# ctSkennerton/crass

Hardware: AMD Instinct MI355X
Metric: reads/sec through DR search+recruit, 150bp synthetic, 1/2/4/8 MI355X (higher is better)
Workload: dtype u8; 1 GPU; 100000000 synthetic 150 bp reads, 50 seeded DRs, 1 % CRISPR reads (BASELINE.json configs[2]); pass1 + merge + pass2; total_reads=100000000, reads_per_gpu=100000000, read_len=150, n_dr=50, parallelism=read-shards x1, launcher=single context, pass1_found=563794, pass2_found=436000, patterns=13320, ac_states=0, filter_survivors=1705594, fast_filter=1, lds_automaton=2, merge_fallbacks=0

## Files before the change

### crass_amd/build.py

```python
import os
import shutil
import subprocess
import sys

HERE = os.path.dirname(os.path.abspath(__file__))
CSRC = os.path.join(HERE, "csrc")
LIB = os.path.join(HERE, "libcrass_hip.so")
SOURCES = ["kernels.hip", "pass2.hip", "sinks.hip", "dmerge.hip", "consensus.hip", "pack.hip", "fastx_scan.hip", "fastx_names.hip", "inflate.hip", "gunzip.hip", "engine.cpp", "engine_pass1.cpp", "engine_merge.cpp", "engine_pass2.cpp", "engine_ingest.cpp", "merge.cpp", "ingest.cpp", "fastx_scan.cpp", "bgzf.cpp", "gunzip.cpp", "consensus.cpp", "group.cpp", "graph.cpp", "sdma.cpp", "pgzip.cpp"]
HEADERS = ["engine_internal.h", "engine_ctx.h", "dev_common.h", "comp_table.h", "devmem.h", "pack_text.h", "lane_find.h", "pack_launch.h", "fastx_scan.h", "fastx_launch.h", "fastx_shards.h", "fastx_names_launch.h", "inflate_core.h", "inflate_launch.h", "gunzip_core.h", "gunzip_launch.h", "consensus_internal.h", "merge.h", os.path.join("..", "..", "include", "crass_hip.h")]


def _hipcc():
    for cand in (os.environ.get("HIPCC"), shutil.which("hipcc"), "/opt/rocm/bin/hipcc"):
        if cand and os.path.exists(cand):
            return cand
    raise RuntimeError("hipcc not found: the MI355X engine cannot be built")


OBJ = os.path.join(CSRC, "_obj")
FLAGS = ["--offload-arch=gfx950", "-O3", "-std=c++17", "-ffp-contract=off", "-fPIC", "-Wall", "-Wno-unused-function"]
LIBS = ["-lz", "-lpthread", "-ldl"]


def _stale(target, deps):
    if not os.path.exists(target):
        return True
    t = os.path.getmtime(target)
    return any(os.path.getmtime(d) > t for d in deps)


def needs_build():
    return _stale(LIB, [os.path.join(CSRC, d) for d in SOURCES + HEADERS])


def build(force=False, verbose=False):
    if not force and not needs_build():
        return LIB
    os.makedirs(OBJ, exist_ok=True)
    hipcc = _hipcc()
    hdrs = [os.path.join(CSRC, h) for h in HEADERS]
    jobs = []
    objs = []
    for s in SOURCES:
        src, obj = os.path.join(CSRC, s), os.path.join(OBJ, s + ".o")
        objs.append(obj)
        if force or _stale(obj, [src] + hdrs):
            cmd = [hipcc] + FLAGS + ["-x", "hip", "-c", src, "-o", obj]
            if verbose:
                print(" ".join(cmd), file=sys.stderr)
            jobs.append((s, subprocess.Popen(cmd, stdout=subprocess.PIPE, stderr=subprocess.STDOUT, text=True)))
    failed = []
    for s, p in jobs:
        out, _ = p.communicate()
        if out.strip():
            print(out, file=sys.stderr, end="")
        if p.returncode:
            failed.append(s)
    if failed:
        raise RuntimeError("hipcc failed for: " + ", ".join(failed))
    tmp = LIB + ".tmp"
    cmd = [hipcc, "--offload-arch=gfx950", "-shared", "-fPIC", "-o", tmp] + objs + LIBS
    if verbose:
        print(" ".join(cmd), file=sys.stderr)
    subprocess.check_call(cmd)
    from . import vgpr_guard
    try:
        vgpr_guard.check(tmp)
    except Exception:
        os.replace(tmp, LIB + ".rejected")
        raise
    os.replace(tmp, LIB)
    return LIB


ADAPTER_DIR = os.path.join(CSRC, "adapter")
CLI = os.path.join(HERE, "crass-hip")
ADAPTER_LIB = os.path.join(HERE, "libcrass_adapter.so")


def build_adapter(force=False, verbose=False):
    build(force=force, verbose=verbose)
    srcs = [os.path.join(ADAPTER_DIR, "crass_adapter.cpp")]
    deps = srcs + [os.path.join(ADAPTER_DIR, "crass_adapter.h"), os.path.join(ADAPTER_DIR, "crass_hip_cli.cpp"), LIB]
    if not force and os.path.exists(CLI) and os.path.exists(ADAPTER_LIB) and \
            all(os.path.getmtime(d) <= min(os.path.getmtime(CLI), os.path.getmtime(ADAPTER_LIB)) for d in deps):
        return CLI
    cxx = shutil.which("g++") or "g++"
    common = [cxx, "-O2", "-std=c++17", "-Wall", "-fPIC", "-pthread"]
    rpath = ["-L" + HERE, "-lcrass_hip", "-Wl,-rpath," + HERE, "-Wl,-rpath,$ORIGIN"]
    for cmd in (common + ["-shared", "-o", ADAPTER_LIB] + srcs + rpath,
                common + ["-o", CLI, os.path.join(ADAPTER_DIR, "crass_hip_cli.cpp")] + srcs + rpath):
        if verbose:
# ... 9 lines not shown
```

### crass_amd/csrc/dev_common.h

```cpp
#pragma once
#include "engine_internal.h"

namespace crass {

#define WAVE 64

static __device__ __forceinline__ void wave_sync()
{
    __builtin_amdgcn_fence(__ATOMIC_RELEASE, "wavefront");
    __builtin_amdgcn_wave_barrier();
    __builtin_amdgcn_fence(__ATOMIC_ACQUIRE, "wavefront");
}

static __device__ __forceinline__ uint32_t uni(uint32_t x) { return (uint32_t)__builtin_amdgcn_readfirstlane((int)x); }
static __device__ __forceinline__ int uni(int x) { return __builtin_amdgcn_readfirstlane(x); }
static __device__ __forceinline__ uint64_t uni64(uint64_t x) { return ((uint64_t)uni((uint32_t)(x >> 32)) << 32) | (uint64_t)uni((uint32_t)x); }

static __device__ __forceinline__ uint64_t rd_word_off(const DevReads &R, uint64_t r)
{
    return R.stride_words ? r * (uint64_t)R.stride_words : R.word_off[r];
}
static __device__ __forceinline__ uint32_t rd_len(const DevReads &R, uint64_t r)
{
    return R.uniform_len ? R.uniform_len : R.lengths[r];
}
static __device__ __forceinline__ bool rd_is_exc(const DevReads &R, uint64_t r)
{
    return (R.exc_mask[r >> 5] >> (r & 31)) & 1u;
}
static __device__ __forceinline__ uint64_t rd_hint_off(const DevReads &R, uint64_t r)
{
    return R.uniform_len ? r * (uint64_t)((R.uniform_len + 63u) >> 6) : R.pos_hint_off[r];
}
static __device__ __forceinline__ uint64_t rd_header_id(const DevReads &R, uint64_t r)
{
    return R.header_id ? R.header_id[r] : r;
}

typedef unsigned short u16x2 __attribute__((ext_vector_type(2)));
static __device__ __forceinline__ uint32_t pk_min_u16(uint32_t a, uint32_t b)
{
    u16x2 r = __builtin_elementwise_min(__builtin_bit_cast(u16x2, a), __builtin_bit_cast(u16x2, b));
    return __builtin_bit_cast(uint32_t, r);
}

}
```

### crass_amd/csrc/dmerge.hip

```cpp
#include "engine_internal.h"
#include <algorithm>

namespace crass {

#define WAVE 64
static constexpr uint32_t kUnres = 0xFFFFFFFFu;
static constexpr uint32_t kNoLane = 0xFFFFFFFEu;
static constexpr int kClusterK = 11;

static __device__ __forceinline__ uint64_t shr128_lo(uint64_t h0, uint64_t h1, uint32_t bits)
{
    if (bits == 0) return h0;
    if (bits < 64) return (h0 >> bits) | (h1 << (64 - bits));
    return h1 >> (bits - 64);
}
static __device__ __forceinline__ uint64_t shr128_hi(uint64_t h1, uint32_t bits)
{
    return bits < 64 ? (h1 >> bits) : 0ull;
}
static __device__ __forceinline__ void mask128(uint32_t len, uint64_t &m0, uint64_t &m1)
{
    if (len >= 32) { m0 = ~0ull; m1 = len >= 64 ? ~0ull : ((1ull << (2 * (len - 32))) - 1ull); }
    else { m0 = (1ull << (2 * len)) - 1ull; m1 = 0ull; }
}
// ... 835 lines not shown

static __device__ __forceinline__ uint32_t dm_rd_len(const DevReads &R, uint64_t r) { return R.uniform_len ? R.uniform_len : R.lengths[r]; }
static __device__ __forceinline__ uint64_t dm_rd_off(const DevReads &R, uint64_t r) { return R.stride_words ? r * (uint64_t)R.stride_words : R.word_off[r]; }

#define DV_MAXW 20
#define DV_G 3
#define DV_GL 21

template <typename WordFn>
static __device__ __forceinline__ void dv_candidates(const DevMerge &M, WordFn word, const uint8_t *raw, uint32_t L, uint32_t a, uint32_t cnt_s,
                                                     uint32_t base_s, int lane, uint32_t &best_end, uint32_t &best_len, uint32_t &best_pid)
{
    for (uint32_t c0 = 0; c0 < cnt_s; c0 += 64) {
        const uint32_t c = c0 + lane;
        uint32_t cand = 0xFFFFFFFFu, cpid = 0;
        if (c < cnt_s) {
            const uint64_t *ent = M.ents + (uint64_t)(base_s + c) * 2;
            const uint64_t *ent2 = M.ents + ((uint64_t)M.ent_cap + base_s + c) * 2;
            const uint64_t e0 = ent[0], e1 = ent[1], f0 = ent2[0], f1 = ent2[1];
            const uint32_t rr = (uint32_t)e0 & 7u, len = ((uint32_t)e0 >> 3) & 0x7Fu;
            if (a >= rr && a - rr + len <= L) {
                const uint32_t start = a - rr;
                const uint32_t w0 = start >> 4, sh = (start & 15u) * 2u;
                uint32_t x[5];
#pragma unroll
                for (int q = 0; q < 5; q++) x[q] = word(w0 + q);
                uint32_t y[4];
#pragma unroll
                for (int q = 0; q < 4; q++) y[q] = sh ? ((x[q] >> sh) | (x[q + 1] << (32 - sh))) : x[q];
                const uint64_t v0 = (uint64_t)y[0] | ((uint64_t)y[1] << 32), v1 = (uint64_t)y[2] | ((uint64_t)y[3] << 32);
                uint64_t m0, m1;
                mask128(len, m0, m1);
                bool eq = (v0 & m0) == e1 && (v1 & m1) == f0;
                const uint64_t e_mask = f1;
                if (eq && raw) {
                    uint64_t rm = 0;
                    bool other = false;
                    for (uint32_t i = 0; i < len; i++) {
                        const uint8_t ch = raw[start + i];
                        if (!((ch == 'A') | (ch == 'C') | (ch == 'G') | (ch == 'T'))) { rm |= 1ull << i; other |= ch != 'N'; }
                    }
                    eq = !other && rm == e_mask;
                } else if (eq) eq = e_mask == 0ull;
                if (eq) { cand = ((start + len) << 8) | (255u - len); cpid = (uint32_t)(e0 >> 32); }
            }
        }
        uint32_t mn = cand;
#pragma unroll
        for (int off = 32; off > 0; off >>= 1) mn = min(mn, (uint32_t)__shfl_xor((int)mn, off));
        if (mn != 0xFFFFFFFFu) {
            const uint32_t e_end = mn >> 8, e_len = 255u - (mn & 0xFFu);
            if (e_end < best_end || (e_end == best_end && e_len > best_len)) {
                const uint64_t who = __ballot(cand == mn);
                best_end = e_end; best_len = e_len;
                best_pid = (uint32_t)__shfl((int)cpid, __ffsll((unsigned long long)who) - 1);
            }
        }
    }
}

static __device__ __forceinline__ void dv_probe(const DevMerge &M, uint32_t V, uint32_t kmask, uint32_t &cnt, uint32_t &base)
{
    const unsigned long long want = (unsigned long long)V | (1ull << 32);
    uint32_t s = kset_hash(V, M.kset_log);
    for (;;) {
        const unsigned long long kk = M.kset_key[s];
        const uint32_t c_s = M.kset_cnt[s], b_s = M.kset_base[s];
        if (kk == 0ull) break;
        if (kk == want) { cnt = c_s; base = b_s; break; }
        s = (s + 1) & kmask;
    }
}

static __device__ __forceinline__ const uint8_t *dv_raw(const DevReads &R, uint64_t r)
{
    if (!(R.n_exc && ((R.exc_mask[r >> 5] >> (r & 31)) & 1u))) return nullptr;
    uint64_t lo = 0, hi = R.n_exc - 1;
    while (lo < hi) { const uint64_t mid = (lo + hi) >> 1; if (R.exc_read[mid] < r) lo = mid + 1; else hi = mid; }
    return R.exc_bytes + R.exc_off[lo];
}

template <bool SHORT, int U>
__global__ __launch_bounds__(256) void k_dm_verify(DevReads R, DevMerge M, const uint64_t *idx, const uint32_t *d_n, uint64_t n_max,
                                                    uint32_t *info_by_slot, uint32_t *pid_by_slot)
{
    __shared__ uint32_t rw_all[4][DV_G][DV_MAXW + 2];
    const int lane = threadIdx.x & 63, wv = threadIdx.x >> 6;
    const uint64_t wave = __builtin_amdgcn_readfirstlane((uint32_t)((blockIdx.x * (uint64_t)blockDim.x + threadIdx.x) >> 6));
    const uint64_t n_waves = ((uint64_t)gridDim.x * blockDim.x) >> 6;
    uint64_t n = *d_n;
    if (n > n_max) n = n_max;
    const uint32_t kmask = (1u << M.kset_log) - 1u;
    if (SHORT) {
        const int gi = lane / DV_GL, pl = lane % DV_GL;
        const uint32_t L = R.uniform_len, nw = (L + 15) >> 4, h_max = (L - 16) >> 3;
        const bool grp = gi < DV_G;
        const uint64_t stride = n_waves * DV_G;
        const int g0 = (grp ? gi : 0) * DV_GL;
        const uint64_t gmask = grp ? (((1ull << DV_GL) - 1ull) << g0) : 0ull;
        uint32_t *rw = rw_all[wv][grp ? gi : 0];
        const ulonglong2 *ents1 = reinterpret_cast<const ulonglong2 *>(M.ents), *ents2 = ents1 + M.ent_cap;
        uint64_t k = wave * DV_G + (uint64_t)gi;
        bool have = grp && k < n;
        uint64_t r = have ? idx[k] : 0;
        uint32_t wreg = (have && (uint32_t)pl < nw) ? R.packed[dm_rd_off(R, r) + pl] : 0u;
        uint64_t k_n = k + stride;
        bool have_n = grp && k_n < n;
        uint64_t r_n = have_n ? idx[k_n] : 0;
        for (uint64_t k0 = wave * DV_G; k0 < n; k0 += stride) {
            if (have && (uint32_t)pl <= nw + 4u) rw[pl] = wreg;
            __builtin_amdgcn_fence(__ATOMIC_RELEASE, "wavefront");
            __builtin_amdgcn_wave_barrier();
            __builtin_amdgcn_fence(__ATOMIC_ACQUIRE, "wavefront");
            const uint32_t wreg_n = (have_n && (uint32_t)pl < nw) ? R.packed[dm_rd_off(R, r_n) + pl] : 0u;
            const uint64_t k_nn = k_n + stride;
            const bool have_nn = grp && k_nn < n;
            const uint64_t r_nn = have_nn ? idx[k_nn] : 0;
            uint32_t cnt = 0, base = 0;
            if (have && (uint32_t)pl <= h_max) {
                const uint32_t wi = (uint32_t)pl >> 1;
                const uint32_t lo = rw[wi], hi = rw[wi + 1];
                dv_probe(M, (pl & 1) ? ((lo >> 16) | (hi << 16)) : lo, kmask, cnt, base);
            }
            const uint8_t *raw = nullptr;
            if (R.n_exc && have) raw = dv_raw(R, r);
            const uint64_t hits_all = __ballot(cnt > 0);
            uint32_t my = grp ? (uint32_t)(hits_all >> (gi * DV_GL)) & ((1u << DV_GL) - 1u) : 0u;
            uint32_t be = 0xFFFFFFFFu, bl = 0, bp = 0;
            while (__ballot(my != 0u)) {
                bool act = my != 0u;
                const int wsrc = act ? __ffs((int)my) - 1 : 0;
                if (act) my &= my - 1u;
                const uint32_t a = 8u * (uint32_t)wsrc;
                if (act && be <= a + 15u) { act = false; my = 0u; }
                const uint32_t cnt_s = (uint32_t)__shfl((int)cnt, g0 + wsrc), base_s = (uint32_t)__shfl((int)base, g0 + wsrc);
                for (uint32_t c0 = 0; __ballot(act && c0 < cnt_s); c0 += U * DV_GL) {
                    uint32_t cand = 0xFFFFFFFFu, cpid = 0;
                    uint32_t cq[U];
                    bool vq[U];
                    ulonglong2 e1[U], e2[U];
#pragma unroll
                    for (int q = 0; q < U; q++) {
                        cq[q] = c0 + (uint32_t)(q * DV_GL + pl);
                        vq[q] = act && cq[q] < cnt_s;
                        const uint32_t ei = vq[q] ? base_s + cq[q] : 0u;
                        e1[q] = ents1[ei]; e2[q] = ents2[ei];
                    }
#pragma unroll
                    for (int q = 0; q < U; q++) {
                        const uint64_t e0 = e1[q].x;
                        const uint32_t rr = (uint32_t)e0 & 7u, len = ((uint32_t)e0 >> 3) & 0x7Fu;
                        if (vq[q] && a >= rr && a - rr + len <= L) {
                            const uint32_t start = a - rr;
                            const uint32_t w0 = start >> 4, sh = (start & 15u) * 2u;
                            uint32_t x[5];
#pragma unroll
                            for (int i = 0; i < 5; i++) x[i] = rw[w0 + i];
                            uint32_t y[4];
#pragma unroll
                            for (int i = 0; i < 4; i++) y[i] = __builtin_amdgcn_alignbit(x[i + 1], x[i], sh);
                            const uint64_t v0 = (uint64_t)y[0] | ((uint64_t)y[1] << 32), v1 = (uint64_t)y[2] | ((uint64_t)y[3] << 32);
                            uint64_t m0, m1;
                            mask128(len, m0, m1);
                            bool eq = (v0 & m0) == e1[q].y && (v1 & m1) == e2[q].x;
                            const uint64_t e_mask = e2[q].y;
                            if (eq && raw) {
                                uint64_t rm = 0;
                                bool other = false;
                                for (uint32_t i = 0; i < len; i++) {
                                    const uint8_t ch = raw[start + i];
                                    if (!((ch == 'A') | (ch == 'C') | (ch == 'G') | (ch == 'T'))) { rm |= 1ull << i; other |= ch != 'N'; }
                                }
                                eq = !other && rm == e_mask;
                            } else if (eq) eq = e_mask == 0ull;
// ... 7 lines not shown
                        uint32_t mn = cand;
#pragma unroll
                        for (int off = 16; off > 0; off >>= 1) {
                            const uint32_t o = (uint32_t)__shfl_down((int)mn, off);
                            if (pl + off < DV_GL) mn = min(mn, o);
                        }
                        mn = (uint32_t)__shfl((int)mn, g0);
                        const uint64_t who = __ballot(cand == mn) & gmask;
                        const uint32_t pid = (uint32_t)__shfl((int)cpid, who ? __ffsll((unsigned long long)who) - 1 : 0);
                        const uint32_t e_end = mn >> 8, e_len = 255u - (mn & 0xFFu);
                        if (e_end < be || (e_end == be && e_len > bl)) { be = e_end; bl = e_len; bp = pid; }
                    }
                }
            }
            if (have && pl == 0) {
                info_by_slot[k] = bl ? ((be << 8) | bl) : 0u;
                pid_by_slot[k] = bp;
            }
            __builtin_amdgcn_wave_barrier();
            k = k_n; have = have_n; r = r_n; wreg = wreg_n;
            k_n = k_nn; have_n = have_nn; r_n = r_nn;
        }
        return;
    }
    uint32_t *rw = rw_all[wv][0];
    for (uint64_t k = wave; k < n; k += n_waves) {
        const uint64_t r = idx[k];
        const uint32_t L = dm_rd_len(R, r);
        const uint32_t *g = R.packed + dm_rd_off(R, r);
        const uint32_t nw = (L + 15) >> 4;
        const bool staged = nw <= DV_MAXW;
        const uint8_t *raw = dv_raw(R, r);
        if (staged) {
            if ((uint32_t)lane < nw) rw[lane] = g[lane];
            if ((uint32_t)lane == nw) rw[lane] = 0u;
            __builtin_amdgcn_fence(__ATOMIC_RELEASE, "wavefront");
            __builtin_amdgcn_wave_barrier();
            __builtin_amdgcn_fence(__ATOMIC_ACQUIRE, "wavefront");
        }
        auto word = [&](uint32_t i) -> uint32_t {
            if (staged) return rw[min(i, nw)];
            return i < nw ? g[i] : 0u;
        };
        uint32_t best_end = 0xFFFFFFFFu, best_len = 0, best_pid = 0;
        const uint32_t KL = M.akey_bases, vmask = akey_mask(M);
        if (L >= KL) {
            const uint32_t ash = M.akey_shift;
            const uint32_t h_max = (L - KL) >> ash;
            for (uint32_t hb = 0; hb <= h_max; hb += 64) {
                if (best_end <= (hb << ash) + KL - 1u) break;
                const uint32_t h = hb + lane;
                uint32_t cnt = 0, base = 0;
                if (h <= h_max) {
                    const uint32_t pos = h << ash, wi = pos >> 4;
                    const uint32_t lo = word(wi), hi = word(wi + 1);
                    dv_probe(M, __builtin_amdgcn_alignbit(hi, lo, (pos & 15u) * 2u) & vmask, kmask, cnt, base);
                }
                uint64_t hits = __ballot(cnt > 0);
                while (hits) {
                    const int src = __ffsll((unsigned long long)hits) - 1;
                    hits &= hits - 1;
                    const uint32_t a = (hb + (uint32_t)src) << ash;
                    if (best_end <= a + KL - 1u) { hits = 0; break; }
                    const uint32_t cnt_s = (uint32_t)__shfl((int)cnt, src), base_s = (uint32_t)__shfl((int)base, src);
                    dv_candidates(M, word, raw, L, a, cnt_s, base_s, lane, best_end, best_len, best_pid);
                }
            }
        }
        if (lane == 0) {
            info_by_slot[k] = best_len ? ((best_end << 8) | best_len) : 0u;
            pid_by_slot[k] = best_pid;
        }
        __builtin_amdgcn_wave_barrier();
    }
}

hipError_t warm_dmerge_module()
{
    hipFuncAttributes a;
    return hipFuncGetAttributes(&a, reinterpret_cast<const void *>(&k_xg_unpack));
}

hipError_t launch_dm_verify(const DevReads &R, const DevMerge &M, const uint64_t *idx, const uint32_t *d_n, uint64_t n_max,
                            uint32_t *info_by_slot, uint32_t *pid_by_slot, hipStream_t st)
{
    if (n_max == 0) return hipSuccess;
    static const bool dv_one = getenv("CRASS_DV_ONE") != nullptr;
    const bool shortr = M.akey_shift == 3 && M.akey_bases == 16 && R.uniform_len >= 16 && ((R.uniform_len - 16) >> 3) < DV_GL && ((R.uniform_len + 15) >> 4) <= DV_MAXW && !dv_one;
    uint64_t nb = shortr ? (n_max + 4 * DV_G - 1) / (4 * DV_G) : (n_max + 3) / 4;
    if (nb > 8192) nb = 8192;
    static const bool dv_pair = getenv("CRASS_DV_SINGLE") == nullptr;
    if (shortr && dv_pair) CRASS_LAUNCH((k_dm_verify<true, 2>), dim3((unsigned)nb), dim3(256), 0, st, R, M, idx, d_n, n_max, info_by_slot, pid_by_slot);
    else if (shortr) CRASS_LAUNCH((k_dm_verify<true, 1>), dim3((unsigned)nb), dim3(256), 0, st, R, M, idx, d_n, n_max, info_by_slot, pid_by_slot);
    else CRASS_LAUNCH((k_dm_verify<false, 1>), dim3((unsigned)nb), dim3(256), 0, st, R, M, idx, d_n, n_max, info_by_slot, pid_by_slot);
    return hipGetLastError();
}

}
```

### crass_amd/csrc/engine.cpp

```cpp
#include "engine_ctx.h"

#include <cstdio>
#include <new>
#include <string>

void crass_hip_ctx::widen_p1() const
{
    P1Dense &D = dense;
    if (D.wide_ready) return;
    (void)wait_bulk();
    const uint64_t n = D.n;
    const uint32_t ss_cap = D.pack_ss_cap, stride = dr_stride;
    const uint8_t *hb = D.h_blob.p;
    const uint16_t *b_replen = (const uint16_t *)(hb + D.lay.replen), *b_ss = (const uint16_t *)(hb + D.lay.ss);
    const uint8_t *b_nss = hb + D.lay.nss, *b_ss8 = hb + D.lay.ss;
    D.w_replen.resize(n); D.w_nss.resize(n); D.w_ss_off.resize(n); D.w_ss.resize(n * (size_t)ss_cap);
    D.w_dr_len.resize(n); D.w_dr.resize(n * (size_t)stride);
    if (D.dr_fallback) (void)hipStreamSynchronize(copy_stream);
    else (void)wait_dx();
    const size_t per_task = 16384;
    host_parallel_for((size_t)((n + per_task - 1) / per_task), 16, [&](size_t t) {
        const uint64_t k0 = t * per_task, k1 = std::min<uint64_t>(n, k0 + per_task);
        for (uint64_t k = k0; k < k1; k++) { D.w_replen[k] = b_replen[k]; D.w_nss[k] = b_nss[k]; D.w_ss_off[k] = k * (uint64_t)ss_cap; }
        if (D.lay.ss_elem == 1) for (uint64_t i = k0 * ss_cap; i < k1 * (uint64_t)ss_cap; i++) D.w_ss[i] = b_ss8[i];
// ... 118 lines not shown
    c->poll_on = getenv("CRASS_NO_POLL") == nullptr;
    if (hipEventCreateWithFlags(&c->ev_gathered, hipEventDisableTiming) != hipSuccess) { delete c; return CRASS_ERR_HIP; }
    if (hipEventCreateWithFlags(&c->ev_premerge, hipEventDisableTiming) != hipSuccess) { delete c; return CRASS_ERR_HIP; }
    c->dma = sdma_create();
    if (c->dma && !getenv("CRASS_DX_PINNED")) {
        for (auto &d : c->dma_dx) d = sdma_create();
        c->dx_via_dma = c->dma_dx[0] && c->dma_dx[1] && c->dma_dx[2];
    }
    (void)warm_dmerge_module();
    *out = c;
    return CRASS_OK;
}

int crass_hip_stream_wait_event(crass_hip_ctx *c, void *event)
{
    if (!c || !event) return CRASS_ERR_INVALID_ARG;
    (void)hipSetDevice(c->device);
    HIPCHK(c, hipStreamWaitEvent(c->stream, (hipEvent_t)event, 0));
    return CRASS_OK;
}

int crass_hip_reload_env(crass_hip_ctx *c)
{
    if (!c) return CRASS_ERR_INVALID_ARG;
    c->env.read();
    g_dev_cap.store(c->env.pool_cap_bytes, std::memory_order_relaxed);
    c->dp.debug_stop = c->env.surv_debug;
    c->dp.find_serial = c->env.lane_find_serial ? 1u : 0u;
    if (c->env.stage_timing >= 0) c->timing_level = c->env.stage_timing;
    c->lb_on = !c->env.no_lookback;
    return CRASS_OK;
}

int crass_hip_set_stage_timing(crass_hip_ctx *c, int level)
{
    if (!c || level < 0 || level > 2) return CRASS_ERR_INVALID_ARG;
    c->timing_level = level;
    return CRASS_OK;
}

int crass_hip_set_host_view(crass_hip_ctx *c, int light)
{
    if (!c || light < 0 || light > 1) return CRASS_ERR_INVALID_ARG;
    quiesce_worker(c);
    c->host_view_light = light != 0;
    if (c->host_view_light) c->dm.M.x_on = 0;
    return CRASS_OK;
}

int crass_hip_set_timing_focus(crass_hip_ctx *c, unsigned kernels)
{
    if (!c || kernels > 7u) return CRASS_ERR_INVALID_ARG;
    c->timing_focus = kernels;
    return CRASS_OK;
}

void crass_hip_destroy(crass_hip_ctx *c)
{
    if (!c) return;
    (void)hipSetDevice(c->device);
    quiesce_worker(c);
    c->worker.stop();
    if (c->stream) (void)hipStreamSynchronize(c->stream);
    if (c->copy_stream) (void)hipStreamSynchronize(c->copy_stream);
    if (c->hint_stream) (void)hipStreamSynchronize(c->hint_stream);
    (void)sdma_wait(c->dma);
    (void)c->wait_dx();
    ingest_free_all(c);
    if (getenv("CRASS_POLL_REPORT")) fprintf(stderr, "[crass_hip] stage-flag polls that ran out of their budget: %u (of %u flags)\n", c->n_poll_timeouts.load(), c->flag_seq);
    c->lb_status.release(); c->lb_ticket.release(); c->h_lb_fail.release(); c->h_flags.release();
    if (c->xchg.ev_counts) (void)hipEventDestroy(c->xchg.ev_counts);
    c->dm.release(); c->h_qblob.release(); c->xchg.send.release(); c->xchg.xinfo.release(); c->xchg.h_xinfo.release();
    c->dd_map.release(); c->dd_dx_chars.release(); c->dd_dx_len.release(); c->dd_dx_hash.release();
    c->h_dmap.release(); c->h_dx_chars.release(); c->h_dx_len.release(); c->h_dx_hash.release();
    if (c->ev_gathered) (void)hipEventDestroy(c->ev_gathered);
    if (c->ev_sink_copies) (void)hipEventDestroy(c->ev_sink_copies);
    for (int q = 0; q < crass_hip_ctx::kHintParts; q++) if (c->ev_hint[q]) (void)hipEventDestroy(c->ev_hint[q]);
    if (c->ev_hint_go) (void)hipEventDestroy(c->ev_hint_go);
    if (c->hint_stream) (void)hipStreamDestroy(c->hint_stream);
    sdma_destroy(c->dma); c->dma = nullptr;
    for (auto &d : c->dma_sink) { sdma_destroy(d); d = nullptr; }
    for (auto &d : c->dma_dx) { sdma_destroy(d); d = nullptr; }
    if (c->ev_premerge) (void)hipEventDestroy(c->ev_premerge);
    if (c->copy_stream) (void)hipStreamDestroy(c->copy_stream);
    c->r_packed.release(); c->r_word_off.release(); c->r_lengths.release(); c->r_header_id.release();
    c->r_exc_mask.release(); c->r_exc_read.release(); c->r_exc_off.release(); c->r_exc_bytes.release();
    c->d_mask.release(); c->d_word_prefix.release(); c->d_block_sums.release(); c->d_idx.release(); c->d_count.release();
    c->d_found.release(); c->d_hit_info.release(); c->d_surv.release(); c->d_dr.release(); c->d_ss_pool.release();
    c->d_ss_used.release(); c->d_rec.release(); c->d_exc_hit.release(); c->d_extra.release();
    c->g_surv.release(); c->g_dr.release(); c->g_ss.release(); c->g_fidx.release(); c->h_count.release(); c->h_surv.release(); c->h_dr.release(); c->h_ss.release(); c->h_idx.release(); c->h_rec.release();
    c->a_go4w.release(); c->a_go16.release(); c->a_go32.release(); c->a_out.release(); c->a_go4.release(); c->dense.release(); c->d_fidx.release(); c->d_pos_hint.release(); c->d_pos_hint_off.release(); c->d_pos_hint_blk.release(); c->d_punt.release(); c->d_redo.release(); c->dd_keys.release(); c->dd_first.release(); c->dd_slot.release(); c->dd_rep.release(); c->dd_hash.release(); c->h_rep.release(); c->h_hash.release(); c->a_anchor.release(); c->d_slot_info.release(); c->d_slot_pid.release(); c->a_out_pid.release(); c->a_pat_token.release();
    for (auto &e : c->ev) if (e) (void)hipEventDestroy(e);
    if (c->stream) (void)hipStreamDestroy(c->stream);
    delete c;
}

int validate_reads(const crass_reads *r)
{
    if (!r) return CRASS_ERR_INVALID_ARG;
    if (r->n_reads && !r->packed) return CRASS_ERR_INVALID_ARG;
    if (!r->stride_words && r->n_reads && !r->word_off) return CRASS_ERR_INVALID_ARG;
    if (!r->uniform_len && r->n_reads && !r->lengths) return CRASS_ERR_INVALID_ARG;
    if (r->n_exceptions && (!r->exc_read || !r->exc_off || !r->exc_bytes)) return CRASS_ERR_INVALID_ARG;
    if (r->uniform_len > CRASS_HIP_MAX_READ_LEN) return CRASS_ERR_UNSUPPORTED;
    return CRASS_OK;
}

int alloc_scratch(crass_hip_ctx *c)
{
    const uint64_t n = c->R.n_reads;
    const uint64_t n_words = std::max<uint64_t>((n + 63) / 64, 1024);
    HIPCHK(c, c->d_mask.ensure(n_words + 1));
    HIPCHK(c, c->d_word_prefix.ensure(n_words + 1));
    HIPCHK(c, c->d_block_sums.ensure((n_words + 255) / 256 + 2));
    HIPCHK(c, c->d_idx.ensure(n + 1));
    HIPCHK(c, c->d_count.ensure(8));
    HIPCHK(c, c->d_found.ensure(n + 1));
    HIPCHK(c, c->d_hit_info.ensure(n + 1));
    HIPCHK(c, c->d_ss_used.ensure(4));
    HIPCHK(c, c->h_count.ensure(32));
    HIPCHK(c, hipMemsetAsync(c->d_found.p, 0, n + 1, c->stream));
    return CRASS_OK;
}

static int setup_pos_hints(crass_hip_ctx *c, const uint32_t *lengths, uint32_t uniform_len, uint64_t n)
{
    c->n_pos_hint_words = 0;
    c->R.pos_hint = nullptr; c->R.pos_hint_off = nullptr; c->R.wave_walk = 0; c->R.hint_all = 0;
    const DevParams &P = c->dp;
    const bool lane_filter = c->R.stride_words >= 4 && c->R.stride_words <= 16;
    c->hint_filter = c->max_len <= c->env.long_min && !lane_filter && !c->env.no_hint_filter;
    c->hint_filter_any = false;
    const bool shifts_ok = P.lowDR + P.lowSp >= 17 && P.highDR + P.highSp <= 127 && P.highDR + P.highSp >= P.lowDR + P.lowSp;
    const bool lattice_hints = P.window == 8 && P.skips == 8 && shifts_ok;
    const bool any_filter = c->hint_filter && !lattice_hints && shifts_ok && P.window >= 6 && P.window <= 9 && P.skips >= 1;
    if ((c->max_len <= c->env.long_min && !c->hint_filter) || n == 0 || !(lattice_hints || any_filter)) return CRASS_OK;
    if (c->env.no_pos_hints) return CRASS_OK;
    std::vector<uint64_t> off(n + 1);
    uint64_t at = 0;
    for (uint64_t i = 0; i < n; i++) { off[i] = at; at += ((uint64_t)(lengths ? lengths[i] : uniform_len) + 63) / 64; }
    off[n] = at;
    HIPCHK(c, c->d_pos_hint_off.ensure(n + 1)); HIPCHK(c, c->d_pos_hint.ensure(at + 1));
    HIPCHK(c, hipMemcpy(c->d_pos_hint_off.p, off.data(), (n + 1) * 8, hipMemcpyHostToDevice));
    c->n_pos_hint_words = at;
    c->hint_filter_any = any_filter;
    c->R.pos_hint = c->d_pos_hint.p; c->R.pos_hint_off = c->d_pos_hint_off.p;
    c->R.hint_all = any_filter ? 1u : 0u;
    c->R.wave_walk = c->max_len > std::min<uint32_t>(c->env.long_min, c->env.wave_walk_min) ? 1u : 0u;
    c->pos_hint_blk = false;
    { const char *hp = getenv("CRASS_HINT_PARTS");
      const int want = hp ? atoi(hp) : 2;
      const bool big = hp ? (n >= 64 && at >= 2048) : (n >= 4096 && at >= (1u << 20));
      c->hint_parts = (big && !c->hint_filter) ? std::min(std::max(want, 1), (int)crass_hip_ctx::kHintParts) : 1; }
    if (c->hint_parts > 1 && !c->hint_stream) {
        int prio_lo = 0, prio_hi = 0;
        (void)hipDeviceGetStreamPriorityRange(&prio_lo, &prio_hi);
        HIPCHK(c, hipStreamCreateWithPriority(&c->hint_stream, hipStreamNonBlocking, getenv("CRASS_HINT_SAME_PRIORITY") ? 0 : prio_lo));
        for (int q = 0; q < crass_hip_ctx::kHintParts; q++) HIPCHK(c, hipEventCreateWithFlags(&c->ev_hint[q], hipEventDisableTiming));
        HIPCHK(c, hipEventCreateWithFlags(&c->ev_hint_go, hipEventDisableTiming));
    }
    for (int q = 0; q <= c->hint_parts; q++) {
        const uint64_t r = q == c->hint_parts ? n : n * (uint64_t)q / (uint64_t)c->hint_parts;
        c->hint_read_split[q] = r;
        c->hint_word_split[q] = q == c->hint_parts ? at : ((off[r] + 255) & ~255ull);
    }
    if (lengths && n <= 0xFFFFFFFFull) {
// ... 206 lines not shown
```

### crass_amd/csrc/engine_ctx.h

```cpp
#pragma once
#include "../../include/crass_hip.h"
#include "engine_internal.h"
#include "merge.h"
#include "fastx_launch.h"

#include <algorithm>
#include <atomic>
#include <chrono>
#include <condition_variable>
#include <cstdint>
#include <cstdlib>
#include <cstring>
#include <functional>
#include <memory>
#include <mutex>
#include <thread>
#include <utility>
#include <vector>

#pragma GCC visibility push(hidden)
namespace crass {

inline double now_ms()
{
// ... 131 lines not shown
    hipError_t elapsed(int a, int b, float *ms) const { return on ? hipEventElapsedTime(ms, ev[a], ev[b]) : hipSuccess; }
    void destroy() { for (auto &e : ev) { if (e) (void)hipEventDestroy(e); e = nullptr; } on = false; }
};

struct LineFetch {
    DevBuf<uint64_t> src, start, off; DevBuf<uint32_t> len; DevBuf<uint8_t> chars;
    PinBuf<uint64_t> h_src, h_off; PinBuf<uint32_t> h_len; PinBuf<uint8_t> h_chars;
    void release_device() { src.release(); start.release(); off.release(); len.release(); chars.release(); }
    void free_all() { release_device(); h_src.release(); h_off.release(); h_len.release(); h_chars.release(); }
};

struct Ingest {
    DevBuf<uint64_t> t_off; DevBuf<uint8_t> t_dev[2]; PinBuf<uint8_t> t_pin[2];
    hipEvent_t ev_t_copy[2] = {nullptr, nullptr}, ev_t_pack[2] = {nullptr, nullptr};
    StageTimer<2> tm_pack;
    float last_pack_ms = 0;
    DevBuf<uint8_t> x_raw, x_text; DevBuf<FxTile> x_tiles; DevBuf<FxBase> x_base; DevBuf<uint64_t> x_tot, x_rec_pos, x_seq_off;
    PinBuf<uint64_t> x_h_tot, x_h_rec_pos, x_h_seq_off;
    StageTimer<2> tm_scan;
    float last_scan_ms = 0;
    DevBuf<uint64_t> z_idx; DevBuf<uint32_t> z_reason; DevBuf<unsigned long long> z_verdict; DevBuf<uint8_t> z_raw, z_text;
    PinBuf<unsigned long long> z_h_verdict;
    StageTimer<2> tm_inflate;
    float last_inflate_ms = 0;
    DevBuf<uint64_t> gz_a64, gz_b64; DevBuf<uint32_t> gz_a32, gz_b32; DevBuf<uint16_t> gz_sym; DevBuf<uint8_t> gz_win;
    DevBuf<uint64_t> gz_ends;
    StageTimer<6> tm_gzip;
    float last_gzip_ms[5] = {0, 0, 0, 0, 0};
    int gzip_on_device = 0;
    DevBuf<uint64_t> f_idx, f_off; DevBuf<uint8_t> f_rc, f_chars;
    PinBuf<uint64_t> f_h_idx, f_h_off; PinBuf<uint8_t> f_h_rc, f_h_chars;
    StageTimer<2> tm_fetch;
    float last_fetch_ms = 0;
    std::vector<uint8_t> f_flags;
    DevBuf<unsigned long long> n_table; DevBuf<uint64_t> n_rec_pos, n_ids, n_ctl; DevBuf<uint32_t> n_long;
    PinBuf<uint64_t> n_h_ctl;
    StageTimer<3> tm_names;
    float last_hid_ms[3] = {0, 0, 0};
    DevBuf<unsigned long long> nt_table; DevBuf<uint64_t> nt_rec_pos;
    bool have_names = false, nt_on_arena = false;
    const uint8_t *nt_bytes = nullptr; uint64_t nt_n_bytes = 0, nt_n_reads = 0, nt_mask = 0;
    DevBuf<uint8_t> nq_names; DevBuf<uint64_t> nq_off, nq_out; DevBuf<uint32_t> nq_long;
    StageTimer<2> tm_find;
    float last_names_ms[2] = {0, 0};
    LineFetch hl, ql;
    DevBuf<uint8_t> fa_arena; uint64_t fa_bytes = 0; bool have_arena = false;
    PinBuf<uint64_t> fa_h_base; PinBuf<int32_t> fa_h_format;
    struct ShardStaged { uint32_t file; uint64_t a, b, off; };
    DevBuf<uint8_t> sh_stage, sh_tail; DevBuf<FxProbe> sh_part; PinBuf<FxProbe> sh_h_part;
    std::vector<ShardStaged> sh_staged;
    std::vector<uint64_t> sh_base;
    uint64_t sh_n_reads = 0; bool sh_scanned = false, sh_loaded = false;
    StageTimer<2> tm_probe;
    float last_probe_ms = 0;
};

}
#pragma GCC visibility pop

using namespace crass;

struct EnvSwitches {
    bool no_lookback = false, no_pos_hints = false, merge_profile = false, no_lane_kernel = false;
    bool host_merge = false, no_speculation = false, exc_separate = false, dm_inject_fail = false, dm_init_late = false;
    bool no_presize = false;
    bool dd_full_table = false;
    bool no_device_view = false;
    bool force_device_view = false;
    bool no_dense_light = false;
    bool no_warm_launch = false;
    uint32_t view_group_cap = 32768;
    uint32_t view_sort_max = 2048;
    uint64_t test_bounds[4] = {0, 0, 0, 0};
    uint32_t row_cap = 256, dm_group_cap = 16384, surv_debug = 0;
    int stage_timing = -1;
    uint64_t pool_cap_bytes = 0;
    bool no_hint_filter = false;
    uint32_t wave_walk_min = 800;
    uint32_t long_min = 2048;
    uint64_t text_chunk_bytes = 64ull << 20;
    bool inflate_hbm_window = true;
    uint32_t hid_hash_bits = 64;
    bool lane_find_serial = false;
    uint32_t probe_blocks = 0;
    void read()
    {
        auto on = [](const char *n) { return getenv(n) != nullptr; };
        no_lookback = on("CRASS_NO_LOOKBACK"); no_pos_hints = on("CRASS_NO_POS_HINTS");
        merge_profile = on("CRASS_MERGE_PROFILE"); no_lane_kernel = on("CRASS_NO_LANE_KERNEL"); host_merge = on("CRASS_HOST_MERGE");
        no_speculation = on("CRASS_NO_SPECULATION"); exc_separate = on("CRASS_EXC_SEPARATE"); dm_init_late = on("CRASS_DM_INIT_LATE");
        dm_inject_fail = on("CRASS_DM_INJECT_FAIL"); no_presize = on("CRASS_NO_PRESIZE"); no_device_view = on("CRASS_NO_DEVICE_VIEW"); dd_full_table = on("CRASS_DD_FULL_TABLE"); force_device_view = on("CRASS_DEVICE_VIEW");
        view_group_cap = 32768; if (const char *e = getenv("CRASS_VIEW_GROUP_CAP")) view_group_cap = (uint32_t)std::max(1, atoi(e));
        view_sort_max = 2048; if (const char *e = getenv("CRASS_VIEW_SORT_MAX")) view_sort_max = (uint32_t)std::min(2048, std::max(64, atoi(e)));
        row_cap = 256; if (const char *e = getenv("CRASS_ROW_CAP")) row_cap = (uint32_t)std::max(1, atoi(e));
        dm_group_cap = 16384; if (const char *e = getenv("CRASS_DM_GROUP_CAP")) dm_group_cap = (uint32_t)std::max(1, atoi(e));
        surv_debug = 0; if (const char *e = getenv("CRASS_SURV_DEBUG")) surv_debug = (uint32_t)atoi(e);
        stage_timing = -1; if (const char *e = getenv("CRASS_STAGE_TIMING")) stage_timing = std::min(2, std::max(0, atoi(e)));
        for (auto &b : test_bounds) b = 0;
        if (const char *e = getenv("CRASS_TEST_BOUNDS")) { int k = 0; for (const char *q = e; *q && k < 4; k++) { test_bounds[k] = (uint64_t)atoll(q); while (*q && *q != ',') q++; if (*q == ',') q++; } }
        no_hint_filter = on("CRASS_NO_HINT_FILTER");
        wave_walk_min = 800; if (const char *e = getenv("CRASS_WAVE_WALK_MIN")) wave_walk_min = (uint32_t)std::max(0, atoi(e));
        long_min = 2048; if (const char *e = getenv("CRASS_LONG_MIN")) long_min = (uint32_t)std::max(0, atoi(e));
        no_warm_launch = getenv("CRASS_NO_WARM_LAUNCH") != nullptr;
        no_dense_light = getenv("CRASS_NO_DENSE_LIGHT") != nullptr;
        text_chunk_bytes = 64ull << 20; if (const char *e = getenv("CRASS_TEXT_CHUNK_BYTES")) text_chunk_bytes = (uint64_t)std::max(1ll, atoll(e));
        inflate_hbm_window = true; if (const char *e = getenv("CRASS_INFLATE_WINDOW")) inflate_hbm_window = strcmp(e, "lds") != 0;
        hid_hash_bits = 64; if (const char *e = getenv("CRASS_HID_TEST_HASH_BITS")) hid_hash_bits = (uint32_t)std::min(64, std::max(0, atoi(e)));
        lane_find_serial = false; if (const char *e = getenv("CRASS_LANE_FIND_SERIAL")) lane_find_serial = atoi(e) != 0;
        probe_blocks = 0; if (const char *e = getenv("CRASS_PROBE_BLOCKS")) probe_blocks = (uint32_t)std::max(0, atoi(e));
        pool_cap_bytes = 0; if (const char *e = getenv("CRASS_POOL_CAP_MB")) pool_cap_bytes = (uint64_t)std::max(1ll, atoll(e)) << 20;
    }
};

struct crass_hip_ctx {
    crass_params prm{};
    EnvSwitches env;
    DevParams dp{};
    int device = 0;
    hipStream_t stream = nullptr;
    mutable int last_hip = 0;

    DevReads R{};
    bool have_reads = false;
    uint64_t read_base = 0;
    uint32_t max_len = 0;
    bool uniform = false;
    DevBuf<uint32_t> r_packed; DevBuf<uint64_t> r_word_off; DevBuf<uint32_t> r_lengths; DevBuf<uint64_t> r_header_id;
    DevBuf<uint32_t> r_exc_mask; DevBuf<uint64_t> r_exc_read; DevBuf<uint64_t> r_exc_off; DevBuf<uint8_t> r_exc_bytes;
    std::vector<uint64_t> h_exc_read;
    std::vector<uint32_t> h_lengths;
    Ingest in;

    DevBuf<uint64_t> d_mask; DevBuf<uint32_t> d_word_prefix; DevBuf<uint32_t> d_block_sums;
    DevBuf<uint64_t> d_idx; DevBuf<uint32_t> d_count; DevBuf<uint8_t> d_found; DevBuf<uint32_t> d_hit_info;
    bool hints_valid = false;
    DevBuf<SurvOut> d_surv; DevBuf<char> d_dr; DevBuf<uint32_t> d_ss_pool; DevBuf<uint32_t> d_ss_used;
    DevBuf<RecruitOut> d_rec; DevBuf<uint32_t> d_exc_hit; DevBuf<uint64_t> d_extra;
    PinBuf<uint32_t> h_count; PinBuf<SurvOut> h_surv; PinBuf<char> h_dr; PinBuf<uint32_t> h_ss; PinBuf<uint64_t> h_idx;
    DevBuf<SurvOut> g_surv; DevBuf<char> g_dr; DevBuf<uint32_t> g_ss;
    PinBuf<RecruitOut> h_rec;
    DevBuf<uint16_t> a_go16; DevBuf<uint32_t> a_go32; DevBuf<uint16_t> a_out; DevBuf<uint16_t> a_go4;
    DevAutomaton A{};
    HostAutomaton H;
    bool full_automaton_uploaded = false;
    DevBuf<uint32_t> a_go4w;
    DevBuf<uint32_t> a_anchor; DevBuf<uint32_t> d_slot_info; DevBuf<uint32_t> d_slot_pid; DevBuf<uint32_t> a_out_pid; DevBuf<uint32_t> a_pat_token;
    bool have_pat_token = false;
    DevAnchors K{};
    bool have_anchors = false;
    bool have_patterns = false;
    uint32_t n_installed_patterns = 0;

    bool have_pass1 = false;
    struct P1List {
        std::vector<uint64_t> read; std::vector<uint8_t> low; std::vector<uint32_t> replen, nss;
        std::vector<uint64_t> ss_off; std::vector<uint32_t, NoInitAlloc<uint32_t>> ss; std::vector<uint16_t> dr_len; std::vector<char, NoInitAlloc<char>> dr;
        void clear() { read.clear(); low.clear(); replen.clear(); nss.clear(); ss_off.clear(); ss.clear(); dr_len.clear(); dr.clear(); }
        void reserve(size_t n, uint32_t stride) { read.reserve(n); low.reserve(n); replen.reserve(n); nss.reserve(n); ss_off.reserve(n); ss.reserve(n * 6); dr_len.reserve(n); dr.reserve(n * stride); }
        size_t size() const { return read.size(); }
    } cand;
    mutable struct P1Dense {
        DevBuf<uint16_t> d_dr_len; DevBuf<char> d_dr;
        uint64_t n = 0;
        bool active = false;
        PinBuf<uint8_t> h_blob; DevBuf<uint8_t> d_blob;
        P1Blob lay{};
        uint32_t pack_ss_cap = 0;
        bool wide_ready = false;
        std::vector<uint32_t> w_replen, w_nss; std::vector<uint32_t, NoInitAlloc<uint32_t>> w_ss; std::vector<uint64_t> w_ss_off; std::vector<uint16_t> w_dr_len;
        std::vector<char, NoInitAlloc<char>> w_dr;
        PinBuf<char> h_dr_fb; PinBuf<uint16_t> h_dr_len_fb; bool dr_fallback = false;
        void release()
        {
            h_blob.release(); d_blob.release(); h_dr_fb.release(); h_dr_len_fb.release(); d_dr_len.release(); d_dr.release();
        }
    } dense;
    DevBuf<uint64_t> d_fidx;
    DevBuf<uint64_t> g_fidx;
    DevBuf<uint64_t> d_pos_hint, d_pos_hint_off; uint64_t n_pos_hint_words = 0;
    DevBuf<uint32_t> d_punt;
    DevBuf<uint32_t> d_redo;
    SdmaCopy *dma_sink[4] = {nullptr, nullptr, nullptr, nullptr};
    DevBuf<uint32_t> d_pos_hint_blk; bool pos_hint_blk = false;
    DevBuf<unsigned long long> dd_keys; DevBuf<uint32_t> dd_first, dd_slot, dd_rep; DevBuf<uint64_t> dd_hash;
    PinBuf<uint32_t> h_rep; PinBuf<uint64_t> h_hash;
    bool have_rep = false;
    DevBuf<uint32_t> dd_map; DevBuf<char> dd_dx_chars; DevBuf<uint16_t> dd_dx_len; DevBuf<uint64_t> dd_dx_hash;
    PinBuf<uint32_t> h_dmap; PinBuf<char> h_dx_chars; PinBuf<uint16_t> h_dx_len; PinBuf<uint64_t> h_dx_hash;
    uint64_t n_dx = 0;
    bool have_dev_tokens = false;
    uint32_t n_cu = 0;
    bool host_view_light = false;
    HostWorker worker;
    uint64_t surv_cap_hint = 0;
    uint64_t hit_cap_hint = 0;
    bool recruit_exact = false;
    hipStream_t copy_stream = nullptr;
    static constexpr int kHintParts = 4;
    hipStream_t hint_stream = nullptr;
    hipEvent_t ev_hint[kHintParts] = {nullptr, nullptr, nullptr, nullptr}, ev_hint_go = nullptr;
    int hint_parts = 1;
    bool hint_filter = false;
    bool hint_filter_any = false;
    uint64_t hint_read_split[kHintParts + 1] = {0, 0, 0, 0, 0}, hint_word_split[kHintParts + 1] = {0, 0, 0, 0, 0};
    DevBuf<uint16_t> g_dr_len; DevBuf<uint64_t> hl_dx_idx;
    bool hint_pending = false;
    hipEvent_t ev_gathered = nullptr;
    hipEvent_t ev_premerge = nullptr;
    mutable bool bulk_pending = false;
    int wait_bulk() const
    {
        if (!bulk_pending) return bulk_status;
        const hipError_t e = hipStreamSynchronize(copy_stream);
        int de = sdma_wait(dma);
        for (SdmaCopy *s : dma_sink) de |= sdma_wait(s);
        bulk_pending = false;
        if (e != hipSuccess) { last_hip = (int)e; bulk_status = CRASS_ERR_HIP; }
        else if (de) { last_hip = (int)hipErrorUnknown; bulk_status = CRASS_ERR_HIP; }
        return bulk_status;
    }
    SdmaCopy *dma = nullptr;
    SdmaCopy *dma_dx[3] = {nullptr, nullptr, nullptr};
    bool dx_via_dma = false;
    mutable std::mutex dx_mu;
    mutable bool dx_pending = false, dx_stream_copy = false;
    mutable int dx_status = CRASS_OK;
    mutable bool dx_hash_valid = true;
    int wait_dx() const
    {
        std::lock_guard<std::mutex> lk(dx_mu);
        if (!dx_pending) return dx_status;
        int bad = 0;
        for (SdmaCopy *s : dma_dx) bad |= sdma_wait(s);
        if (dx_stream_copy) { const hipError_t e = hipStreamSynchronize(copy_stream); if (e != hipSuccess) { last_hip = (int)e; bad = 1; } }
        dx_pending = false; dx_stream_copy = false;
        if (bad) { if (!last_hip) last_hip = (int)hipErrorUnknown; dx_status = CRASS_ERR_HIP; }
        return dx_status;
    }
    mutable int bulk_status = CRASS_OK;
    struct DM {
        DevBuf<uint64_t> packed, tmask; DevBuf<uint32_t> codes, owner, root_of, pat_token;
        DevBuf<uint32_t> kset_u32, ent_slot, anchor_tab, anchor_fp; DevBuf<uint8_t> blank; DevBuf<uint64_t> ents, rents; DevBuf<uint32_t> rset_u32, rd_slot;
        DevBuf<unsigned long long> rset_key, bk_key;
        DevBuf<unsigned long long> kset_key; DevBuf<DevMergeState> st; DevBuf<uint32_t> hot;
        PinBuf<DevMergeState> h_st; PinBuf<uint32_t> h_root; PinBuf<uint8_t> h_blank;
        std::vector<uint32_t> gid_tmp;
        DevMerge M{};
        bool active = false, host_built = false;
        int build_status = 0;
        bool build_pending = false;
        struct BuildResult { bool valid = false; uint32_t n_patterns = 0, n_keys = 0; float ms_device = 0; int hip = 0; } br;
        uint64_t n_cand = 0;
        const char *hx_chars = nullptr; const uint16_t *hx_len = nullptr; uint64_t n_tok = 0;
        bool global = false; uint64_t my_off = 0, n_global = 0;
        DevBuf<char> g_chars, gx_chars; DevBuf<uint16_t> g_len, gx_len; DevBuf<unsigned long long> g_keys;
        DevBuf<uint32_t> g_first, g_slot, g_rep, g_prefix, g_bsum; DevBuf<uint64_t> g_hash, g_mask, g_idx;
        PinBuf<uint32_t> h_gmap; PinBuf<char> h_gx_chars; PinBuf<uint16_t> h_gx_len; PinBuf<uint64_t> h_gx_hash;
        std::vector<uint32_t> cand_map;
        hipEvent_t ev_done = nullptr, ev_t0 = nullptr, ev_t1 = nullptr;
        uint32_t want_post = 0;
        DevBuf<uint32_t> x_u32, x_members, x_tile; DevBuf<uint8_t> x_blob; DevBuf<DevViewTotals> x_tot;
        PinBuf<DevViewTotals> x_htot; PinBuf<uint8_t> h_view;
        hipStream_t view_stream = nullptr; hipEvent_t ev_fork = nullptr, ev_view = nullptr, ev_apply = nullptr;
        SdmaCopy *dma_view = nullptr, *dma_view2 = nullptr, *dma_view3 = nullptr;
        uint32_t want_blank = 0;
        bool hx_on_host = true;
        bool view_launched = false;
        bool apply_recorded = false;
        bool view_ready = false;
        DevViewTotals view_tot{};
        void release()
        {
            x_u32.release(); x_members.release(); x_tile.release(); x_blob.release(); x_tot.release(); x_htot.release(); h_view.release();
            packed.release(); tmask.release(); bk_key.release(); codes.release(); owner.release(); root_of.release();
            pat_token.release(); kset_u32.release(); ent_slot.release(); anchor_tab.release(); anchor_fp.release();
            blank.release(); ents.release(); rents.release(); rset_u32.release(); rd_slot.release(); rset_key.release(); kset_key.release(); st.release(); hot.release(); h_st.release(); h_root.release(); h_blank.release();
            g_chars.release(); gx_chars.release(); g_len.release(); gx_len.release(); g_keys.release(); g_first.release(); g_slot.release();
            g_rep.release(); g_prefix.release(); g_bsum.release(); g_hash.release(); g_mask.release(); g_idx.release();
            h_gmap.release(); h_gx_chars.release(); h_gx_len.release(); h_gx_hash.release();
            if (ev_done) (void)hipEventDestroy(ev_done);
// ... 189 lines not shown
```

### crass_amd/csrc/engine_internal.h

```cpp
#pragma once
#include <stdint.h>
#include <stddef.h>
#include <hip/hip_runtime.h>
#include "devmem.h"
#include "merge.h"

namespace crass {

struct DevReads {
    const uint32_t *packed;
    const uint64_t *word_off;
    const uint32_t *lengths;
    const uint64_t *header_id;
    const uint32_t *exc_mask;
    uint64_t n_reads;
    uint32_t stride_words;
    uint32_t uniform_len;
    const uint64_t *exc_read;
    const uint64_t *exc_off;
    const uint8_t  *exc_bytes;
    uint64_t n_exc;
    const uint64_t *pos_hint;
    const uint64_t *pos_hint_off;
    uint32_t wave_walk;
// ... 121 lines not shown
    uint32_t *rd_slot;
    uint64_t *rents;
    uint32_t *pat_token;
    const uint64_t *pat_mask;
    unsigned long long *kset_key;
    uint32_t *kset_cnt, *kset_base, *kset_fill;
    uint32_t kset_log;
    uint32_t *ent_slot;
    uint64_t *ents;
    uint32_t ent_cap;
    uint32_t *anchor_tab;
    uint32_t *anchor_fp;
    uint32_t tab_log_alloc;
    uint32_t m1, m2;
    uint32_t n_cu;
    DevMergeState *st;
    DevMergeState *h_st; uint32_t *h_root; uint8_t *h_blank;
    uint32_t *x_size, *x_kept, *x_kchars, *x_fill;
    uint32_t *x_gid, *x_goff, *x_pat0, *x_pch0;
    uint32_t *x_members;
    uint32_t *x_tile;
    uint8_t  *x_blob;
    DevViewTotals *x_tot;
    DevViewTotals *x_htot;
    uint32_t x_on;
    uint32_t x_group_cap;
    uint32_t *flag_pre; uint32_t flag_pre_val;
    uint32_t *flag_post; uint32_t flag_post_val;
    uint32_t *flag_blank; uint32_t flag_blank_val;
    uint32_t x_sort_max;
    uint32_t *hot;
    uint32_t ablate;
    uint32_t inject_fail;
    uint32_t group_cap;
    uint32_t akey_bases;
};

static __device__ __forceinline__ void dm_init_slice(const DevMerge &M, uint64_t tid, uint64_t nth)
{
    uint4 ones; ones.x = ones.y = ones.z = ones.w = 0xFFFFFFFFu;
    uint4 *o4 = reinterpret_cast<uint4 *>(M.owner);
    for (uint64_t i = tid; i < ((1u << 22) + kDmBadSlots) / 4; i += nth) o4[i] = ones;
    for (uint64_t i = tid; i < kDmBadSlots; i += nth) M.bk_key[i] = 0ull;
    for (uint64_t i = tid; i < M.n_tok; i += nth) M.root_of[i] = 0xFFFFFFFFu;
    if (M.x_on) {
        for (uint64_t i = tid; i < M.n_tok; i += nth) { M.x_size[i] = 0u; M.x_kept[i] = 0u; M.x_kchars[i] = 0u; M.x_fill[i] = 0u; }
        if (tid < 4) M.x_tile[kDmxTiles * kDmxVals + tid] = 0u;
    }
    const uint64_t ks = 1ull << M.kset_log;
    for (uint64_t i = tid; i < ks; i += nth) { M.kset_key[i] = 0ull; M.kset_cnt[i] = 0u; M.kset_fill[i] = 0u; }
    const uint64_t rs = 1ull << M.rset_log;
    for (uint64_t i = tid; i < rs; i += nth) { M.rset_key[i] = 0ull; M.rset_cnt[i] = 0u; M.rset_fill[i] = 0u; }
    for (uint64_t i = tid; i < (1u << 15); i += nth) M.anchor_fp[i] = 0u;
    uint4 *t4 = reinterpret_cast<uint4 *>(M.anchor_tab);
    for (uint64_t i = tid; i < (1ull << M.tab_log_alloc) / 4; i += nth) t4[i] = ones;
    if (tid < kDmHotStripes) {
        M.hot[dm_hot(kHotSurvivors, (uint32_t)tid)] = 0u; M.hot[dm_hot(kHotKeys, (uint32_t)tid)] = 0u; M.hot[dm_hot(kHotK0, (uint32_t)tid)] = 0xFFFFFFFFu;
        M.hot[dm_hot(kHotEntCursor, (uint32_t)tid)] = 0u; M.hot[dm_hot(kHotRdCursor, (uint32_t)tid)] = 0u;
    }
    if (tid == 0) {
        DevMergeState s{};
        s.k0 = 0xFFFFFFFFu;
        s.fail = M.inject_fail ? 16u : 0u;
        *M.st = s;
    }
}

static __device__ __forceinline__ void stage_flag_store(uint32_t *flag, uint32_t val)
{
    __hip_atomic_store(flag, val, __ATOMIC_RELEASE, __HIP_MEMORY_SCOPE_SYSTEM);
}
hipError_t launch_xg_fill(const char *dx_chars, const uint16_t *dx_len, const uint32_t *d_nd, uint32_t stride, uint64_t cap_rows,
                          uint32_t slot_bytes, uint8_t *send, hipStream_t st, const uint32_t *p1_counts = nullptr, uint64_t surv_bound = 0,
                          uint32_t *h_flag = nullptr, uint32_t flag_val = 0);
hipError_t launch_xg_unpack(const uint8_t *recv, uint32_t world, uint32_t rank, uint32_t stride, uint64_t cap_rows, uint32_t slot_bytes,
                            char *g_chars, uint16_t *g_len, uint32_t *xinfo, hipStream_t st, uint32_t *h_xinfo = nullptr,
                            uint32_t *zero2 = nullptr,
                            unsigned long long *dd_keys = nullptr, uint32_t *dd_first = nullptr, uint32_t dd_size = 0);
hipError_t launch_device_merge(const DevMerge &M, hipStream_t st, bool init_done = false, hipStream_t view_st = nullptr,
                               hipEvent_t ev_fork = nullptr, hipEvent_t ev_view = nullptr,
                               hipEvent_t ev_apply = nullptr);
hipError_t launch_anchor_filter_dev(const DevReads &R, const DevMerge &M, const uint8_t *found_flag, uint64_t *hitmask, hipStream_t st, uint32_t max_blocks = 0);
hipError_t launch_dm_verify(const DevReads &R, const DevMerge &M, const uint64_t *idx, const uint32_t *d_n, uint64_t n_max,
                            uint32_t *info_by_slot, uint32_t *pid_by_slot, hipStream_t st);
hipError_t warm_dmerge_module();

struct SurvLds {
    uint32_t seq_bytes;
    uint32_t ss_cap;
    uint32_t row_elems;
    uint32_t words_cap;
    uint32_t hint_words;
    uint32_t total_bytes;
    uint32_t seq_window;
    uint32_t ss_slot;
};

hipError_t launch_filter_general(const DevReads &R, const DevParams &P, uint64_t *hitmask,
                                 uint32_t max_len, hipStream_t st);
hipError_t launch_hint_positions(const DevReads &R, const DevParams &P, const uint64_t *hint_off, const uint32_t *blk_read, uint64_t n_words,
                                 uint64_t *hint_bits, hipStream_t st,
                                 uint64_t w_begin = 0, uint64_t w_end = ~0ull,
                                 uint64_t *hitmask = nullptr);
hipError_t launch_hint_filter_any(const DevReads &R, const DevParams &P, const uint64_t *hint_off, const uint32_t *blk_read, uint64_t n_words,
                                  uint64_t *hitmask, uint64_t *hint_bits, hipStream_t st);
hipError_t launch_long_light(const DevReads &R, const DevParams &P, const uint32_t *d_n, uint64_t n_max, SurvOut *out, uint64_t slot_base,
                             uint32_t max_len, hipStream_t st, uint32_t *punt_list, uint32_t *d_punt_n, const uint64_t *surv_idx = nullptr);
hipError_t launch_filter_fast(const DevReads &R, const DevParams &P, uint64_t *hitmask, uint32_t *seed_hint, hipStream_t st,
                              uint8_t *clear_found = nullptr, bool *cleared = nullptr);
#define CRASS_VGPR_FLOOR(N) asm volatile("" ::: "v" #N)

#ifdef __HIPCC__
template <int THREADS>
static __device__ __forceinline__ uint32_t block_reserve(uint32_t v, uint32_t *counter)
{
    __shared__ uint32_t br_tot[THREADS / 64];
    __shared__ uint32_t br_base;
    const int lane = threadIdx.x & 63, w = threadIdx.x >> 6;
    uint32_t incl = v;
#pragma unroll
    for (int off = 1; off < 64; off <<= 1) {
        const uint32_t u = (uint32_t)__shfl_up((int)incl, off);
        if (lane >= off) incl += u;
    }
    if (lane == 63) br_tot[w] = incl;
    __syncthreads();
    if (threadIdx.x == 0) {
        uint32_t tot = 0;
        for (int i = 0; i < THREADS / 64; i++) { const uint32_t x = br_tot[i]; br_tot[i] = tot; tot += x; }
        br_base = tot ? atomicAdd(counter, tot) : 0u;
    }
    __syncthreads();
    return br_base + br_tot[w] + incl - v;
}
#endif

struct Lookback {
    unsigned long long *status;
    uint32_t *ticket;
    uint32_t epoch;
    uint32_t *fail;
};
static inline uint32_t lookback_tile_words(uint64_t n_words) { return n_words >= 16384 ? 4096u : 256u; }

hipError_t launch_compact(const uint64_t *mask, uint64_t n_words, uint64_t n_bits, uint32_t *word_prefix,
                          uint32_t *block_sums, uint64_t *out_idx, uint64_t out_cap, uint32_t *d_count,
                          hipStream_t st, uint32_t *zero_a = nullptr, uint32_t n_a = 0, uint32_t *zero_b = nullptr, uint32_t n_b = 0,
                          const Lookback *lb = nullptr);
hipError_t launch_survivor(const DevReads &R, const DevParams &P, bool exceptions,
                           const uint64_t *surv_idx, const uint32_t *d_n_surv, uint64_t n_surv_max,
                           SurvOut *out, char *dr_chars, uint32_t dr_stride,
                           uint32_t *ss_pool, uint32_t ss_pool_cap, uint32_t *d_ss_used,
                           uint8_t *found_flag, const uint32_t *seed_hint, const SurvLds &lds, int grid, hipStream_t st,
                           int punt_only = 0,
                           uint64_t slot_base = 0, uint64_t slot_total = 0,
                           const uint32_t *punt_list = nullptr, const uint32_t *d_punt_n = nullptr,
                           uint32_t *redo_list = nullptr);
hipError_t launch_survivor_lanes(const DevReads &R, const DevParams &P, const uint64_t *surv_idx, const uint32_t *d_n_surv,
                                 uint64_t n_surv_max, SurvOut *out, char *dr_chars, uint32_t dr_stride, uint32_t *ss_pool,
                                 uint32_t ss_cap, uint8_t *found_flag, const uint32_t *seed_hint, hipStream_t st,
                                 const DevMerge *init_merge = nullptr, uint32_t max_len = 0, uint32_t *punt_cnt = nullptr);
hipError_t launch_recruit_general(const DevReads &R, const DevAutomaton &A, const uint8_t *found_flag,
                                  uint64_t *hitmask, uint32_t *hit_info, hipStream_t st);
hipError_t launch_recruit_lds(const DevReads &R, const DevAutomaton &A, const uint8_t *found_flag,
                              uint64_t *hitmask, uint32_t *hit_info, hipStream_t st);
hipError_t launch_anchor_filter(const DevReads &R, const DevAnchors &K, const uint8_t *found_flag,
                                uint64_t *hitmask, hipStream_t st, uint32_t max_blocks = 0);
hipError_t launch_recruit_list(const DevReads &R, const DevAutomaton &A, const uint64_t *idx, const uint32_t *d_n,
                               uint64_t n_max, uint32_t *info_by_slot, uint32_t *pid_by_slot, hipStream_t st);
hipError_t launch_recruit_exceptions(const DevReads &R, const DevAutomaton &A, const uint8_t *found_flag,
                                     uint32_t *exc_hit_info , hipStream_t st);
hipError_t launch_recruit_finish(const DevReads &R, const uint64_t *hit_idx, const uint32_t *d_n_hits,
                                 uint64_t n_hits_max, const uint32_t *hit_info, bool info_by_slot, bool exceptions,
                                 const uint32_t *pid_by_slot, const uint32_t *pat_token,
                                 RecruitOut *out, char *dr_chars, uint32_t dr_stride, hipStream_t st,
                                 const uint64_t *pat_mask = nullptr);
hipError_t launch_levenshtein_batch(const uint8_t *chars, const uint64_t *a_off, const uint32_t *a_len,
                                    const uint64_t *b_off, const uint32_t *b_len, uint64_t n_pairs,
                                    int32_t *dist, float *sim, uint32_t max_len, hipStream_t st);
hipError_t launch_mark_found(const uint64_t *idx, uint64_t n, const uint64_t *header_id, uint8_t *found_flag, hipStream_t st);
hipError_t launch_copy_to_host(const void *d_src, void *h_dst, uint64_t bytes, hipStream_t st);
struct SdmaCopy;
SdmaCopy *sdma_create();
void sdma_destroy(SdmaCopy *s);
bool sdma_start(SdmaCopy *s, const void *d_src, void *h_dst, size_t bytes);
int sdma_wait(SdmaCopy *s);
bool sdma_pending(const SdmaCopy *s);
hipError_t launch_build_exc_mask(const uint64_t *exc_read, uint64_t n_exc, uint32_t *exc_mask, hipStream_t st);

hipError_t launch_found_compact(const SurvOut *out, const uint32_t *d_n, uint64_t n_max, uint32_t *d_err, unsigned long long *dd_keys,
                                uint32_t *dd_first, uint32_t dd_size, uint64_t *fidx, uint32_t *d_nf, const Lookback &lb, hipStream_t st);
hipError_t launch_select_found(const SurvOut *out, uint64_t n, uint64_t *mask, uint32_t *d_err, hipStream_t st);
hipError_t launch_gather_sparse(const uint64_t *fidx, const uint32_t *d_nf, uint64_t n_max, const SurvOut *out, const char *dr_chars, uint32_t dr_stride,
                                const uint32_t *ss_pool, SurvOut *g_out, uint64_t *g_slot, char *g_dr, uint32_t *g_ss, uint32_t g_ss_cap,
                                uint32_t *d_ss_total, hipStream_t st, uint16_t *g_dr_len = nullptr,
                                int ss16 = 0);
hipError_t launch_found_mask(const SurvOut *out, const uint32_t *d_n, uint64_t n, uint64_t *mask, uint32_t *d_err, hipStream_t st,
                             unsigned long long *dd_keys = nullptr, uint32_t *dd_first = nullptr, uint32_t dd_size = 0);
hipError_t launch_gather_found(const uint64_t *fidx, const uint32_t *d_nf, uint64_t n_max, const SurvOut *out,
                               const uint64_t *surv_idx, uint64_t read_base, const char *dr_chars, uint32_t dr_stride,
                               const uint32_t *ss_pool, uint32_t ss_cap, uint32_t ss_elem, uint8_t *blob,
                               uint16_t *g_dr_len, char *g_dr, hipStream_t st,
                               unsigned long long *dd_keys = nullptr, uint32_t *dd_first = nullptr, uint32_t dd_size = 0,
                               uint64_t *dd_hash = nullptr, uint32_t *dd_slot = nullptr, uint32_t *d_mismatch = nullptr);
static constexpr uint32_t kDdMaxProbes = 256;
struct P1Blob { uint64_t read, replen, nss, low, ss, total; uint32_t ss_elem; };
__host__ __device__ inline P1Blob p1_blob_layout(uint64_t nf, uint32_t ss_cap, uint32_t ss_elem = 2)
{
    P1Blob b;
    uint64_t at = 0;
    auto sec = [&](uint64_t bytes) { const uint64_t o = at; at += (bytes + 15u) & ~15ull; return o; };
    b.read = sec(nf * 8); b.replen = sec(nf * 2); b.nss = sec(nf); b.low = sec(nf); b.ss = sec(nf * (uint64_t)ss_cap * ss_elem);
    b.total = at; b.ss_elem = ss_elem;
    return b;
}
struct P2Blob { uint64_t read, token, start, end, dr_len, low, total; uint32_t narrow; };
__host__ __device__ inline P2Blob p2_blob_layout(uint64_t cap, uint32_t narrow = 0)
{
    P2Blob b;
    uint64_t at = 16;
    auto sec = [&](uint64_t bytes) { const uint64_t o = at; at += (bytes + 15u) & ~15ull; return o; };
    b.read = sec(cap * (narrow ? 4 : 8)); b.token = sec(cap * 4); b.start = sec(cap * (narrow ? 1 : 2));
    if (narrow == 2) { b.end = at; b.dr_len = at; b.low = at; }
    else { b.end = sec(cap * (narrow ? 1 : 2)); b.dr_len = sec(cap); b.low = sec(cap); }
    b.total = at; b.narrow = narrow;
    return b;
}
hipError_t launch_pack_p2_blob(const RecruitOut *rec, const uint64_t *hit_idx, uint64_t read_base,
                               const uint32_t *d_n_hits, uint64_t n_hits_max, uint64_t *mask, uint32_t *word_prefix, uint32_t *block_sums,
                               uint64_t *vidx, uint32_t *d_nv, uint8_t *blob, hipStream_t st,
                               uint32_t *h_n_hits = nullptr,
                               const Lookback *lb = nullptr, uint32_t narrow = 0);
hipError_t launch_dx_tokens(const char *dr, const uint16_t *dr_len, const uint64_t *hash, uint32_t stride, const uint32_t *d_n, uint32_t n, uint32_t *rep,
                            uint32_t *slot_of, const uint32_t *first,
                            uint64_t *mask, uint32_t *word_prefix, uint32_t *block_sums, uint64_t *dx_idx, uint32_t *d_nd,
                            uint32_t *d_mismatch, uint32_t *dmap, char *out_chars, uint16_t *out_len, uint64_t *out_hash,
                            char *dev_chars, uint16_t *dev_len, hipStream_t st,
                            const uint32_t *cnt_src = nullptr, uint32_t *cnt_dst = nullptr, uint32_t n_cnt = 0,
                            const Lookback *lb = nullptr);
hipError_t launch_dr_dedupe(const char *dr, const uint16_t *dr_len, uint32_t stride, const uint32_t *d_n, uint32_t n, unsigned long long *keys,
                            uint32_t *first, uint32_t table_size, uint64_t *hash_out, uint32_t *slot_tmp, uint32_t *rep, hipStream_t st,
                            bool table_cleared = false);
SurvLds survivor_lds_layout(uint32_t max_len, const DevParams &P, uint32_t row_len_cap = 0xFFFFFFFFu,
                            uint32_t seq_window_bytes = 0, uint32_t ss_entries_cap = 0);

}
```

### crass_amd/csrc/engine_pass1.cpp

```cpp
#include "engine_ctx.h"

#include <cstdio>

extern "C" {

static int hint_wait_all(crass_hip_ctx *c)
{
    if (!c->hint_pending) return CRASS_OK;
    HIPCHK(c, hipStreamWaitEvent(c->stream, c->ev_hint[c->hint_parts - 1], 0));
    c->hint_pending = false;
    return CRASS_OK;
}

static bool getenv_once_hl_host() { static const bool v = getenv("CRASS_HL_HOST_DEDUPE") != nullptr; return v; }
static bool getenv_once_copy_early() { static const bool on = getenv("CRASS_COPY_EARLY") != nullptr; return on; }

static void dump_surv_prof(crass_hip_ctx *c)
{
    if (!c->dp.prof) return;
    unsigned long long v[192];
    if (hipMemcpy(v, c->dp.prof, sizeof v, hipMemcpyDeviceToHost) != hipSuccess) return;
    (void)hipMemset(c->dp.prof, 0, sizeof v);
    { const unsigned long long big = ~0ull; (void)hipMemcpy(c->dp.prof + 188, &big, 8, hipMemcpyHostToDevice); }
    if (v[191]) fprintf(stderr, "[surv_prof] %llu waves; first start .. last start %.1f us, first start .. last end %.1f us\n", v[186], (double)(v[187] - v[188]) / 100.0, (double)(v[189] - v[188]) / 100.0);
// ... 431 lines not shown
        if (!lattice && !c->R.hint_all) RL.pos_hint = nullptr;
        HIPCHK(c, c->d_punt.ensure(n_surv + 1)); HIPCHK(c, hipMemsetAsync(c->d_punt.p, 0, 4, c->stream));
        const hipError_t ll = launch_long_light(RL, c->dp, d_nsurv, n_surv, c->d_surv.p, 0, c->max_len, c->stream, c->d_punt.p + 1, c->d_punt.p, c->d_idx.p);
        if (ll == hipSuccess) {
            light_done = true;
            HIPCHK(c, launch_survivor(c->R, c->dp, false, c->d_idx.p, d_nsurv, n_surv, c->d_surv.p, c->d_dr.p, stride,
                                      c->d_ss_pool.p, (uint32_t)pool_cap, c->d_ss_used.p, c->d_found.p, hints, lds,
                                      (int)std::min<uint64_t>(256 * 12, n_surv), c->stream, 7, 0, 0, c->d_punt.p + 1, c->d_punt.p));
        } else if (ll != hipErrorNotSupported) { c->last_hip = (int)ll; return CRASS_ERR_HIP; }
    }
    if (!light_done)
    HIPCHK(c, launch_survivor(c->R, c->dp, false, c->d_idx.p, d_nsurv, n_surv, c->d_surv.p, c->d_dr.p, stride,
                              c->d_ss_pool.p, (uint32_t)pool_cap, c->d_ss_used.p, c->d_found.p, hints, lds,
                              (int)std::min<uint64_t>(256 * 32, n_surv), c->stream, le == hipSuccess ? 4 : 0, 0, 0, nullptr,
                              le == hipSuccess ? c->d_count.p + 6 : nullptr));
    if (c->R.n_exc)
        HIPCHK(c, launch_survivor(c->R, c->dp, true, c->d_idx.p, d_nsurv, n_surv, c->d_surv.p, c->d_dr.p, stride,
                                  c->d_ss_pool.p, (uint32_t)pool_cap, c->d_ss_used.p, c->d_found.p, nullptr, lds,
                                  (int)std::min<uint64_t>(256 * 32, n_surv), c->stream, 5));
    HIPCHK(c, c->stamp(9, 1));
    const uint64_t n_words = (n_surv + 63) / 64;
    uint32_t tsize = 1024;
    if (dedupe) while (tsize < n_surv * 2) tsize <<= 1;
    if (dedupe && speculative && c->dx_cap_hint && !c->dd_full_table && !c->env.dd_full_table) {
        uint32_t small = c->env.test_bounds[1] ? 64u : 4096u;
        while (small < c->dx_cap_hint * 4ull && small < tsize) small <<= 1;
        tsize = std::min(tsize, small);
    }
    Lookback lbf;
    if (const Lookback *lb = c->next_lookback_elems(n_surv, &lbf)) {
        HIPCHK(c, launch_found_compact(c->d_surv.p, d_nsurv, n_surv, c->d_count.p + 3, dedupe ? c->dd_keys.p : nullptr,
                                       dedupe ? c->dd_first.p : nullptr, tsize, c->d_fidx.p, c->d_count.p + 2, *lb, c->stream));
    } else {
        HIPCHK(c, launch_found_mask(c->d_surv.p, d_nsurv, n_surv, c->d_mask.p, c->d_count.p + 3, c->stream,
                                    dedupe ? c->dd_keys.p : nullptr, dedupe ? c->dd_first.p : nullptr, tsize));
        HIPCHK(c, launch_compact(c->d_mask.p, n_words, n_surv, c->d_word_prefix.p, c->d_block_sums.p, c->d_fidx.p, n_surv, c->d_count.p + 2, c->stream));
    }
    HIPCHK(c, launch_gather_found(c->d_fidx.p, c->d_count.p + 2, n_surv, c->d_surv.p, c->d_idx.p, c->read_base, c->d_dr.p, stride,
                                  c->d_ss_pool.p, lds.ss_cap, ss_elem, D.d_blob.p, D.d_dr_len.p, D.d_dr.p, c->stream,
                                  dedupe ? c->dd_keys.p : nullptr, dedupe ? c->dd_first.p : nullptr, tsize, c->dd_hash.p, c->dd_slot.p,
                                  c->d_count.p + 5));
    c->have_rep = false;
    c->have_dev_tokens = false;
    if (dedupe) {
        Lookback lbd;
        const bool dxd = c->dx_via_dma;
        HIPCHK(c, launch_dx_tokens(D.d_dr.p, D.d_dr_len.p, c->dd_hash.p, stride, c->d_count.p + 2, (uint32_t)n_surv, c->dd_rep.p, c->dd_slot.p, c->dd_first.p, c->d_mask.p,
                                   c->d_word_prefix.p, c->d_block_sums.p, c->d_fidx.p, c->d_count.p + 4, c->d_count.p + 5, dxd ? c->dd_map.p : c->h_dmap.p,
                                   dxd ? nullptr : c->h_dx_chars.p, dxd ? nullptr : c->h_dx_len.p, dxd ? nullptr : c->h_dx_hash.p, c->dd_dx_chars.p, c->dd_dx_len.p, c->stream,
                                   c->d_count.p, defer_ok ? c->h_count.p + 16 : c->h_count.p, 8,
                                   c->next_lookback_tiles((n_surv + 1023) / 1024, &lbd)));
        if (c->xchg.active)
            HIPCHK(c, launch_xg_fill(c->dd_dx_chars.p, c->dd_dx_len.p, c->d_count.p + 4, stride, c->xchg.cap, c->xchg.slot, c->xchg.send.p, c->stream,
                                     defer_ok ? c->d_count.p : nullptr, n_surv,
                                     (defer_ok && c->poll_on) ? c->h_flags.p : nullptr, (defer_ok && c->poll_on) ? (c->want_p1 = ++c->flag_seq) : 0u));
    }
    if (!dedupe) HIPCHK(c, hipMemcpyAsync(c->h_count.p, c->d_count.p, 32, hipMemcpyDeviceToHost, c->stream));
    bool premerge_queued = false;
    c->premerge = 0;
    D.wide_ready = false; D.dr_fallback = false;
    D.pack_ss_cap = lds.ss_cap;
    const bool will_premerge = speculative && dedupe && !c->xchg.active && c->dm_prev_local && c->dx_cap_hint && c->prm.lowDRsize >= (int)kDevMinDR && stride <= 64 &&
                               !c->env.host_merge && !c->env.no_speculation;
    if (!c->poll_on && (will_premerge || defer_ok)) HIPCHK(c, hipEventRecord(c->ev_gathered, c->stream));
    if (will_premerge) {
        const bool prepared = c->dm_prepared_n == c->dx_cap_hint && c->dm_prepared_src == c->dd_dx_chars.p;
        const int ps = device_merge_enqueue(c, c->dd_dx_chars.p, c->dd_dx_len.p, c->dx_cap_hint, c->d_count.p + 4, prepared);
        if (ps) return ps;
        premerge_queued = true;
        if (!c->poll_on || !c->dma) HIPCHK(c, hipEventRecord(c->ev_premerge, c->stream));
    }
    host_pool_warm();
    if (defer_ok) {
        c->p1d.active = true; c->p1d.n_bound = n_surv; c->p1d.ss_cap = lds.ss_cap; c->p1d.ss_elem = ss_elem;
        return CRASS_OK;
    }
    return dense_after_sync(c, n_surv, lds.ss_cap, ss_elem, dedupe, premerge_queued, overflow);
}

int ensure_recruit_buffers(crass_hip_ctx *c, uint64_t h_alloc, uint64_t n_exc, bool dev_sink, bool anchors)
{
    const uint64_t s_alloc = h_alloc + n_exc;
    { const int ms = ensure_mask_scratch(c, h_alloc); if (ms) return ms; }
    HIPCHK(c, c->d_rec.ensure(s_alloc + 1));
    HIPCHK(c, c->d_dr.ensure((s_alloc + 1) * c->dr_stride));
    if (!dev_sink) {
        HIPCHK(c, c->h_rec.ensure(s_alloc + 1));
        HIPCHK(c, c->h_dr.ensure((s_alloc + 1) * c->dr_stride));
        HIPCHK(c, c->h_idx.ensure(h_alloc + 1));
    }
    if (anchors) {
        HIPCHK(c, c->d_slot_info.ensure(h_alloc + 1));
        HIPCHK(c, c->d_slot_pid.ensure(h_alloc + 1));
    }
    if (dev_sink) {
        HIPCHK(c, c->h_qblob.ensure(p2_blob_layout(h_alloc).total + 64));
        HIPCHK(c, c->d_fidx.ensure(h_alloc + 1));
    }
    return CRASS_OK;
}

static int first_call_bounds_impl(crass_hip_ctx *c)
{
    c->surv_cap_hint = 0; c->hit_cap_hint = 0; c->dx_cap_hint = 0; c->dm_prev_local = false; c->premerge = 0;
    c->recruit_exact = false;
    const uint64_t n = c->R.n_reads;
    if (c->env.no_presize || c->env.no_speculation || n == 0 || c->max_len > c->env.long_min) return CRASS_OK;
    if (c->R.n_exc && c->env.exc_separate) return CRASS_OK;
    const DevParams &P = c->dp;
    const SurvLds lds = survivor_lds_layout(c->max_len, P);
    if (lds.total_bytes > 160 * 1024 || lds.ss_cap > 128 || (c->dr_stride & 15)) return CRASS_OK;
    const uint32_t min_len = P.lowDR + P.lowSp + P.window + 1;
    const double seeds = c->max_len > min_len ? (double)(c->max_len - min_len) / P.skips + 1.0 : 1.0;
    const double cand = (double)(P.highDR + P.highSp - P.lowDR - P.lowSp + 1);
    double rate = seeds * cand / (double)(1ull << (2 * P.window)) + 0.02;
    if (rate > 1.0) rate = 1.0;
    uint64_t surv = survivor_bound((uint64_t)((double)n * rate));
    if (surv > n + 65536) surv = survivor_bound(n * 2 / 3);
    if (c->env.test_bounds[0]) surv = std::max<uint64_t>(64, c->env.test_bounds[0]);
    const uint64_t pool_cap = std::max<uint64_t>(surv * (uint64_t)lds.ss_cap, 1u << 16);
    if (surv > kDenseMaxSurvivors || pool_cap >= (1ull << 31)) return CRASS_OK;
    size_t free_b = 0, total_b = 0;
    if (hipMemGetInfo(&free_b, &total_b) != hipSuccess) return CRASS_OK;
    const uint64_t per = 140ull + 3ull * c->dr_stride + 6ull * lds.ss_cap;
    if (surv * per > free_b / 4) return CRASS_OK;
    const bool dedupe = surv < (1u << 24);
    int s = ensure_dense_buffers(c, surv, pool_cap, lds, dedupe);
    if (s) return s;
    c->surv_cap_hint = surv;
    { const uint64_t nw = (n + 63) / 64; c->prealloc_lookback(std::max<uint64_t>((nw + lookback_tile_words(nw) - 1) / lookback_tile_words(nw), (surv + 1023) / 1024)); }
    if (dedupe && c->prm.lowDRsize >= (int)kDevMinDR && c->dr_stride <= 64 && !c->env.host_merge) {
        uint64_t dx = crass_hip_exchange_rows_for(n);
        if (c->env.test_bounds[1]) dx = std::max<uint64_t>(16, c->env.test_bounds[1]);
        s = device_merge_prepare(c, c->dd_dx_chars.p, c->dd_dx_len.p, dx, c->d_count.p + 4);
        if (s) return s;
        c->dx_cap_hint = (uint32_t)dx;
        c->dm_prev_local = true;
        try {
            auto touch = [](auto &v, size_t k) { v.resize(k); v.clear(); };
            MergeResult &m = c->merge;
            touch(m.cand_token, (size_t)(n / 128 + 4096));
            touch(m.tokens.strings.chars, (size_t)dx * 48); touch(m.tokens.strings.off, (size_t)dx + 2); m.tokens.strings.clear();
            touch(m.patterns.chars, (size_t)dx * 24); touch(m.patterns.off, (size_t)dx + 2); m.patterns.clear();
            touch(m.pat_group, (size_t)dx); touch(m.pat_token, (size_t)dx); touch(m.grp_tokens, (size_t)dx); touch(m.grp_off, (size_t)dx / 4 + 16);
        } catch (const std::bad_alloc &) { }
    }
    uint64_t hits = hit_bound(n / 64);
    if (c->env.test_bounds[2]) hits = std::max<uint64_t>(16, c->env.test_bounds[2]);
    s = ensure_recruit_buffers(c, hits, 0, true, true);
    if (s) return s;
    c->hit_cap_hint = hits;
    if (!c->env.no_warm_launch) {
        HIPCHK(c, hipMemsetAsync(c->d_count.p, 0, 32, c->stream));
        HIPCHK(c, launch_survivor(c->R, c->dp, false, c->d_idx.p, c->d_count.p + 1, surv, c->d_surv.p, c->d_dr.p, c->dr_stride,
                                  c->d_ss_pool.p, (uint32_t)pool_cap, c->d_ss_used.p, c->d_found.p, nullptr, lds,
                                  (int)std::min<uint64_t>(256 * 32, surv), c->stream, 4));
    }
    host_pool_warm();
    return CRASS_OK;
}

int first_call_bounds(crass_hip_ctx *c)
{
    const int s = first_call_bounds_impl(c);
    if (s == CRASS_ERR_OOM) {
        c->surv_cap_hint = 0; c->hit_cap_hint = 0; c->dx_cap_hint = 0; c->dm_prev_local = false; c->premerge = 0;
        c->last_hip = 0;
// ... 264 lines not shown
```

### crass_amd/csrc/engine_pass2.cpp

```cpp
#include "engine_ctx.h"

#include <cstdio>

extern "C" {

int crass_hip_set_patterns(crass_hip_ctx *c, const char *const *patterns, const uint32_t *lengths, uint32_t n)
{
    if (!c || (n && (!patterns || !lengths))) return CRASS_ERR_INVALID_ARG;
    StringArena pats;
    for (uint32_t i = 0; i < n; i++) pats.push(patterns[i], lengths[i]);
    c->have_pass2 = false;
    return install_patterns(c, pats);
}

static int recruit_after_host_merge(crass_hip_ctx *c, const uint64_t *extra_found, uint64_t n_extra)
{
    if (const int fs = host_merge_fallback(c)) return fs;
    return crass_hip_recruit(c, extra_found, n_extra);
}

static int mark_extra_found(crass_hip_ctx *c, const uint64_t *extra_found, uint64_t n_extra)
{
    for (uint64_t i = 0; i < n_extra; i++) if (extra_found[i] >= c->R.n_reads) return CRASS_ERR_INVALID_ARG;
    HIPCHK(c, c->d_extra.ensure(n_extra));
    HIPCHK(c, hipMemcpyAsync(c->d_extra.p, extra_found, n_extra * 8, hipMemcpyHostToDevice, c->stream));
    HIPCHK(c, launch_mark_found(c->d_extra.p, n_extra, c->R.header_id, c->d_found.p, c->stream));
    HIPCHK(c, hipStreamSynchronize(c->stream));
    return CRASS_OK;
}

static int launch_probe(crass_hip_ctx *c, bool dmp, uint64_t n_exc, bool &anchors, bool &lds)
{
    anchors = lds = false;
    if (dmp) {
        HIPCHK(c, launch_anchor_filter_dev(c->R, c->dm.M, c->d_found.p, c->d_mask.p, c->stream, c->env.probe_blocks));
        anchors = true;
    } else if (c->have_anchors) {
        hipError_t ae = launch_anchor_filter(c->R, c->K, c->d_found.p, c->d_mask.p, c->stream, c->env.probe_blocks);
        if (ae == hipSuccess) anchors = true;
        else if (ae != hipErrorNotSupported) { c->last_hip = (int)ae; return CRASS_ERR_HIP; }
    }
    if (!anchors || n_exc) { int fs = ensure_full_automaton(c); if (fs) return fs; }
    if (!anchors) {
        hipError_t re = launch_recruit_lds(c->R, c->A, c->d_found.p, c->d_mask.p, c->d_hit_info.p, c->stream);
        lds = (re == hipSuccess);
        if (re == hipErrorNotSupported) { HIPCHK(c, launch_recruit_general(c->R, c->A, c->d_found.p, c->d_mask.p, c->d_hit_info.p, c->stream)); }
        else if (re != hipSuccess) { c->last_hip = (int)re; return CRASS_ERR_HIP; }
    }
    if (n_exc) {
        HIPCHK(c, c->d_exc_hit.ensure(n_exc));
        HIPCHK(c, launch_recruit_exceptions(c->R, c->A, c->d_found.p, c->d_exc_hit.p, c->stream));
    }
    return CRASS_OK;
}

static int recruit_device_sink(crass_hip_ctx *c, bool spec, uint64_t n_hits, const uint64_t *extra_found, uint64_t n_extra)
{
    static const bool blob12 = getenv("CRASS_P2_BLOB12") != nullptr;
    const uint32_t narrow = (c->max_len <= 255 && c->R.n_reads < (1ull << 32)) ? ((blob12 || c->host_view_light) ? 1u : 2u) : 0u;
    c->q_lay = p2_blob_layout(n_hits, narrow);
    c->q_wide_ready = false;
    Lookback lbq;
    if (n_hits) {
        HIPCHK(c, launch_pack_p2_blob(c->d_rec.p, c->d_idx.p, c->read_base, c->d_count.p, n_hits, c->d_mask.p,
                                      c->d_word_prefix.p, c->d_block_sums.p, c->d_fidx.p, c->d_count.p + 6, c->h_qblob.p, c->stream,
                                      spec ? c->h_count.p : nullptr, c->next_lookback_elems(n_hits, &lbq), narrow));
    } else memset(c->h_qblob.p, 0, 16);
    const double th0 = now_ms();
    const int hs = ensure_host_merge(c);
    c->cnt.ms_merge_host += (float)(now_ms() - th0);
    if (c->env.merge_profile)
        fprintf(stderr, "[crass_dm] recruit: tail queued %.1f us after the pass-1 sync, then blocked %.1f us on the host view\n",
                1e3 * (th0 - c->t_p1_sync), 1e3 * (now_ms() - th0));
    if (hs == CRASS_ERR_STATE) {
        HIPCHK(c, hipStreamSynchronize(c->stream));
        return recruit_after_host_merge(c, extra_found, n_extra);
    }
    if (hs) return hs;
    HIPCHK(c, hipStreamSynchronize(c->stream));
    if (c->env.merge_profile)
        fprintf(stderr, "[crass_dm] recruit: final synchronisation returned %.1f us after the pass-1 sync\n", 1e3 * (now_ms() - c->t_p1_sync));
    if (spec) {
        if (c->dm.h_st.p->fail) return recruit_after_host_merge(c, extra_found, n_extra);
        if (c->h_count.p[0] > n_hits) {
            c->n_bound_overflows[2]++;
            c->hit_cap_hint = 0;
            c->recruit_exact = true;
            return crass_hip_recruit(c, extra_found, n_extra);
        }
    }
    c->hit_cap_hint = hit_bound(c->h_count.p[0]);
    if (c->env.merge_profile)
        fprintf(stderr, "[crass_dm] recruit: anchor probe flagged %u of %llu reads (%u keys of %u bases, windows every %u)\n", c->h_count.p[0],
                (unsigned long long)c->R.n_reads, c->dm.h_st.p->n_keys, c->dm.M.akey_bases, 1u << c->dm.M.akey_shift);
    if (const int bs = c->wait_bulk()) return bs;
    c->q_n = *reinterpret_cast<const uint64_t *>(c->h_qblob.p);
    c->q_blob_active = true;
    c->have_pass2 = true;
    c->cnt.n_pass2_found = c->q_n;
    c->cnt.used_lds_automaton = 2;
    c->cnt.anchor_keys = c->dm.h_st.p->n_keys;
    c->cnt.anchor_table_kind = c->dm.h_st.p->tab_mode == 3 ? 1 : c->dm.h_st.p->tab_mode;
    c->spans_p2 = true;
    return c->lookback_ok();
}

static int recruit_host_sink(crass_hip_ctx *c, uint64_t n_hits, uint64_t n_exc, bool anchors, bool lds)
{
    const uint64_t n_slots = n_hits + n_exc;
    if (n_slots) {
        HIPCHK(c, hipMemcpyAsync(c->h_rec.p, c->d_rec.p, n_slots * sizeof(RecruitOut), hipMemcpyDeviceToHost, c->stream));
        HIPCHK(c, hipMemcpyAsync(c->h_dr.p, c->d_dr.p, n_slots * c->dr_stride, hipMemcpyDeviceToHost, c->stream));
    }
    if (n_hits) HIPCHK(c, hipMemcpyAsync(c->h_idx.p, c->d_idx.p, n_hits * 8, hipMemcpyDeviceToHost, c->stream));
    HIPCHK(c, hipStreamSynchronize(c->stream));
    const double t0 = now_ms();
    size_t ia = 0, ib = 0;
    const size_t nb = n_exc;
    auto exc_valid = [&](size_t b) { return c->h_rec.p[n_hits + b].dr_len != 0; };
    while (ib < nb && !exc_valid(ib)) ib++;
    auto hit_valid = [&](size_t a) { return c->h_rec.p[a].dr_len != 0; };
    while (ia < n_hits && !hit_valid(ia)) ia++;
    c->q_dr.reserve(n_slots * c->dr_stride);
    c->q_read.reserve(n_slots); c->q_low.reserve(n_slots); c->q_start.reserve(n_slots); c->q_end.reserve(n_slots);
    c->q_dr_len.reserve(n_slots); c->q_token.reserve(n_slots);
    while (ia < n_hits || ib < nb) {
        const bool takeA = ib >= nb || (ia < n_hits && c->h_idx.p[ia] < c->h_exc_read[ib]);
        const size_t slot = takeA ? ia : n_hits + ib;
        const RecruitOut &o = c->h_rec.p[slot];
        const uint64_t r = takeA ? c->h_idx.p[ia] : c->h_exc_read[ib];
        c->q_read.push_back(c->read_base + r); c->q_low.push_back(o.low_lexi);
        c->q_start.push_back(o.start); c->q_end.push_back(o.end); c->q_dr_len.push_back(o.dr_len);
        const char *dr = c->h_dr.p + slot * c->dr_stride;
        const size_t at = c->q_dr.size();
        c->q_dr.resize(at + c->dr_stride);
        memset(c->q_dr.data() + at, 0, c->dr_stride);
        memcpy(c->q_dr.data() + at, dr, o.dr_len);
        uint32_t tok = o.token;
        if (!tok && c->have_merge) {
            tok = c->merge.tokens.get(dr, o.dr_len);
            if (!tok) tok = c->merge.tokens.add(dr, o.dr_len);
        }
        c->q_token.push_back(tok);
        if (takeA) { ia++; while (ia < n_hits && !hit_valid(ia)) ia++; }
        else { ib++; while (ib < nb && !exc_valid(ib)) ib++; }
    }
    c->have_pass2 = true;
    c->cnt.ms_sink_host += (float)(now_ms() - t0);
    c->cnt.n_pass2_found = c->q_read.size();
    c->cnt.used_lds_automaton = anchors ? 2 : (lds ? 1 : 0);
    c->cnt.anchor_keys = anchors ? c->K.n_keys : 0;
    c->cnt.anchor_table_kind = anchors ? (c->K.log_size > 15 ? 2 : c->K.mode) : 0;
    c->spans_p2 = true;
    return c->lookback_ok();
}

int crass_hip_recruit(crass_hip_ctx *c, const uint64_t *extra_found, uint64_t n_extra)
{
    if (!c) return CRASS_ERR_INVALID_ARG;
    if (!c->have_reads) return CRASS_ERR_STATE;
    (void)hipSetDevice(c->device);
    if (c->p1d.active) { const int ds = settle_p1(c); if (ds) return ds; }
    c->q_read.clear(); c->q_low.clear(); c->q_start.clear(); c->q_end.clear(); c->q_token.clear(); c->q_dr_len.clear(); c->q_dr.clear();
    c->have_pass2 = false;
    c->q_blob_active = false;
    c->cnt.n_pass2_found = 0;
    if (c->n_installed_patterns == 0) { c->have_pass2 = true; return CRASS_OK; }
    if (!c->have_patterns) return CRASS_ERR_STATE;
    const uint64_t n = c->R.n_reads;
    const uint64_t n_words = (n + 63) / 64;
    if (n_extra) { const int ms = mark_extra_found(c, extra_found, n_extra); if (ms) return ms; }
    HIPCHK(c, c->stamp(5, 1));
    const bool dmp = c->dm.active;
    const uint64_t n_exc = dmp ? 0 : c->R.n_exc;
    bool anchors = false, lds = false;
    if (const int ps = launch_probe(c, dmp, n_exc, anchors, lds)) return ps;
    HIPCHK(c, c->stamp(6, 1));
    Lookback lbr;
    HIPCHK(c, launch_compact(c->d_mask.p, n_words, n, c->d_word_prefix.p, c->d_block_sums.p, c->d_idx.p, n, c->d_count.p, c->stream,
                             nullptr, 0, nullptr, 0, c->next_lookback(n_words, &lbr)));
    const bool spec = dmp && c->hit_cap_hint && !c->env.no_speculation && !c->recruit_exact;
    c->recruit_exact = false;
    if (!spec) { const int rs = read_count(c); if (rs) return rs; }
    if (!spec && dmp && c->dm.h_st.p->fail) return recruit_after_host_merge(c, extra_found, n_extra);
    const uint64_t n_hits = spec ? c->hit_cap_hint : c->h_count.p[0];
    const uint64_t h_alloc = spec ? n_hits : std::max<uint64_t>(n_hits, hit_bound(n_hits));
    { const int as = ensure_recruit_buffers(c, h_alloc, n_exc, dmp, anchors); if (as) return as; }
    if (anchors) {
        if (dmp) HIPCHK(c, launch_dm_verify(c->R, c->dm.M, c->d_idx.p, c->d_count.p, n_hits, c->d_slot_info.p, c->d_slot_pid.p, c->stream));
        else HIPCHK(c, launch_recruit_list(c->R, c->A, c->d_idx.p, c->d_count.p, n_hits, c->d_slot_info.p, c->d_slot_pid.p, c->stream));
    }
    const bool dev_tokens = dmp || (anchors && c->have_pat_token && c->have_merge);
    HIPCHK(c, launch_recruit_finish(c->R, c->d_idx.p, c->d_count.p, n_hits, anchors ? c->d_slot_info.p : c->d_hit_info.p, anchors, false,
                                    dev_tokens ? c->d_slot_pid.p : nullptr, dev_tokens ? (dmp ? c->dm.M.pat_token : c->a_pat_token.p) : nullptr,
                                    c->d_rec.p, dmp ? nullptr : c->d_dr.p, c->dr_stride, c->stream, dmp ? c->dm.M.pat_mask : nullptr));
    if (n_exc)
        HIPCHK(c, launch_recruit_finish(c->R, nullptr, nullptr, n_exc, c->d_exc_hit.p, true, true, nullptr, nullptr, c->d_rec.p + n_hits,
                                        c->d_dr.p + n_hits * c->dr_stride, c->dr_stride, c->stream));
    HIPCHK(c, c->stamp(7, 2));
    if (dmp) return recruit_device_sink(c, spec, n_hits, extra_found, n_extra);
    return recruit_host_sink(c, n_hits, n_exc, anchors, lds);
}

int crass_hip_get_recruits(const crass_hip_ctx *c, crass_recruits *o)
{
    if (!c || !o) return CRASS_ERR_INVALID_ARG;
    if (!c->have_pass2) return CRASS_ERR_STATE;
    if (c->q_blob_active && !c->q_wide_ready) {
        crass_hip_ctx *mc = const_cast<crass_hip_ctx *>(c);
        const uint8_t *hb = c->h_qblob.p;
        const P2Blob &b = c->q_lay;
        const uint64_t n = c->q_n;
        const uint32_t *b_tok = (const uint32_t *)(hb + b.token);
        const uint16_t *b_start = (const uint16_t *)(hb + b.start), *b_end = (const uint16_t *)(hb + b.end);
        mc->q_read.resize(n); mc->q_token.resize(n); mc->q_low.resize(n);
        mc->q_start.resize(n); mc->q_end.resize(n); mc->q_dr_len.resize(n); mc->q_dr.resize(n * (size_t)c->dr_stride);
        const bool dv = c->dm.active && c->dm.view_ready;
        const uint8_t *vb = c->dm.h_view.p;
        const uint64_t *v_off = dv ? (const uint64_t *)(vb + c->dm.view_tot.lay.tok_off) : nullptr;
        const char *v_chars = dv ? (const char *)(vb + c->dm.view_tot.lay.tok_chars) : nullptr;
        const uint32_t n_tok = dv ? c->dm.view_tot.n_tok : c->merge.tokens.size();
        const size_t per_task = 16384;
        const size_t stride = c->dr_stride;
        host_parallel_for((size_t)((n + per_task - 1) / per_task), 16, [&](size_t task) {
            const uint64_t k0 = task * per_task, k1 = std::min<uint64_t>(n, k0 + per_task);
            memset(mc->q_dr.data() + k0 * stride, 0, (size_t)(k1 - k0) * stride);
            for (uint64_t k = k0; k < k1; k++) {
                mc->q_read[k] = b.narrow ? c->read_base + ((const uint32_t *)(hb + b.read))[k] : ((const uint64_t *)(hb + b.read))[k];
                const uint32_t t = b.narrow == 2 ? (b_tok[k] & 0x7FFFFFFFu) : b_tok[k];
                mc->q_token[k] = t;
                size_t tlen = 0;
                if (t >= 2 && t - 2 < n_tok) {
                    tlen = dv ? (size_t)(v_off[t - 1] - v_off[t - 2]) : (size_t)c->merge.tokens.strings.len(t - 2);
                    if (dv) memcpy(mc->q_dr.data() + k * stride, v_chars + v_off[t - 2], tlen);
                    else memcpy(mc->q_dr.data() + k * stride, c->merge.tokens.strings.data(t - 2), tlen);
                }
                if (b.narrow == 2) {
                    mc->q_low[k] = (uint8_t)(b_tok[k] >> 31);
                    mc->q_start[k] = (hb + b.start)[k];
                    mc->q_dr_len[k] = (uint16_t)tlen;
                    mc->q_end[k] = mc->q_start[k] + (tlen ? (uint32_t)tlen - 1u : 0u);
                    continue;
                }
                mc->q_low[k] = (hb + b.low)[k];
                if (b.narrow) { mc->q_start[k] = (hb + b.start)[k]; mc->q_end[k] = (hb + b.end)[k]; }
                else { mc->q_start[k] = b_start[k]; mc->q_end[k] = b_end[k]; }
                mc->q_dr_len[k] = (hb + b.dr_len)[k];
            }
        });
        mc->q_wide_ready = true;
    }
    o->n = c->q_read.size(); o->read_idx = c->q_read.data(); o->low_lexi = c->q_low.data();
    o->start = c->q_start.data(); o->end = c->q_end.data(); o->dr_stride = c->dr_stride;
    o->dr_len = c->q_dr_len.data(); o->dr_chars = c->q_dr.data(); o->token = c->q_token.data();
    return CRASS_OK;
}

}
```

### crass_amd/csrc/pass2.hip

```cpp
#include "dev_common.h"
#include "comp_table.h"
#include <type_traits>
#include <utility>

namespace crass {

static __constant__ CompTable c_comp = make_comp_table();

template <bool LDS_TABLE, int THREADS>
__global__ __launch_bounds__(THREADS) void k_recruit(DevReads R, DevAutomaton A, const uint8_t *found_flag,
                                                 uint64_t *hitmask, uint32_t *hit_info)
{
    extern __shared__ __attribute__((aligned(16))) uint16_t rc_lds[];
    const uint16_t *go4 = A.go4;
    const uint16_t *outl = A.out_len;
    if (LDS_TABLE) {
        uint16_t *l_go = rc_lds;
        uint16_t *l_out = rc_lds + (size_t)A.n_states * 4;
        for (uint32_t i = threadIdx.x; i < A.n_states * 4; i += blockDim.x) l_go[i] = A.go4[i];
        for (uint32_t i = threadIdx.x; i < A.n_states; i += blockDim.x) l_out[i] = A.out_len[i];
        __syncthreads();
        go4 = l_go; outl = l_out;
    }
    const uint64_t n_tiles = (R.n_reads + 63) / 64;
    const int lane = threadIdx.x & 63;
    const uint64_t wave_global = (blockIdx.x * (uint64_t)blockDim.x + threadIdx.x) >> 6;
    const uint64_t wave_total = ((uint64_t)gridDim.x * blockDim.x) >> 6;
    for (uint64_t tile = wave_global; tile < n_tiles; tile += wave_total) {
        const uint64_t r = tile * 64 + lane;
        bool hit = false;
        if (r < R.n_reads && !rd_is_exc(R, r) && !found_flag[rd_header_id(R, r)]) {
            const uint32_t L = rd_len(R, r);
            const uint32_t *g = R.packed + rd_word_off(R, r);
            uint32_t state = 0;
            uint32_t word = 0;
            for (uint32_t i = 0; i < L; i++) {
                if ((i & 15u) == 0) word = g[i >> 4];
                uint32_t c = word & 3u;
                word >>= 2;
                state = go4[state * 4 + c];
                uint32_t ol = outl[state];
                if (ol) { hit_info[r] = ((i + 1) << 8) | ol; hit = true; break; }
            }
        }
        uint64_t m = __ballot(hit);
        if (lane == 0) hitmask[tile] = m;
    }
}

__global__ __launch_bounds__(256) void k_recruit_wide(DevReads R, DevAutomaton A, const uint8_t *found_flag,
                                                       uint64_t *hitmask, uint32_t *hit_info)
{
    const uint64_t n_tiles = (R.n_reads + 63) / 64;
    const int lane = threadIdx.x & 63;
    const uint64_t wave_global = (blockIdx.x * (uint64_t)blockDim.x + threadIdx.x) >> 6;
    const uint64_t wave_total = ((uint64_t)gridDim.x * blockDim.x) >> 6;
    const uint32_t symA = A.sym['A'], symC = A.sym['C'], symG = A.sym['G'], symT = A.sym['T'];
    for (uint64_t tile = wave_global; tile < n_tiles; tile += wave_total) {
        const uint64_t r = tile * 64 + lane;
        bool hit = false;
        if (r < R.n_reads && !rd_is_exc(R, r) && !found_flag[rd_header_id(R, r)]) {
            const uint32_t L = rd_len(R, r);
            const uint32_t *g = R.packed + rd_word_off(R, r);
            uint32_t state = 0, word = 0;
            for (uint32_t i = 0; i < L; i++) {
                if ((i & 15u) == 0) word = g[i >> 4];
                uint32_t c = word & 3u;
                word >>= 2;
                uint32_t sy = c == 0 ? symA : c == 1 ? symC : c == 2 ? symG : symT;
                state = A.go16 ? (uint32_t)A.go16[(size_t)state * A.n_sym1 + sy] : A.go32[(size_t)state * A.n_sym1 + sy];
                uint32_t ol = A.out_len[state];
                if (ol) { hit_info[r] = ((i + 1) << 8) | ol; hit = true; break; }
            }
        }
        uint64_t m = __ballot(hit);
        if (lane == 0) hitmask[tile] = m;
    }
}

hipError_t launch_recruit_general(const DevReads &R, const DevAutomaton &A, const uint8_t *found_flag,
                                  uint64_t *hitmask, uint32_t *hit_info, hipStream_t st)
{
    if (R.n_reads == 0) return hipSuccess;
    uint64_t n_tiles = (R.n_reads + 63) / 64;
    uint64_t blocks = (n_tiles + 3) / 4;
    if (blocks > 256 * 8) blocks = 256 * 8;
    if (A.acgt_ok && A.go4)
        CRASS_LAUNCH((k_recruit<false, 256>), dim3((unsigned)blocks), dim3(256), 0, st, R, A, found_flag, hitmask, hit_info);
// ... 360 lines not shown
                                                            uint64_t n_max, uint32_t *info_by_slot, uint32_t *pid_by_slot)
{
    const int lane = threadIdx.x & 63;
    const uint64_t k = (blockIdx.x * (uint64_t)blockDim.x + threadIdx.x) >> 6;
    uint64_t n = *d_n;
    if (n > n_max) n = n_max;
    if (k >= n) return;
    const uint64_t r = idx[k];
    const uint32_t L = rd_len(R, r);
    const uint32_t *g = R.packed + rd_word_off(R, r);
    const uint32_t symA = A.sym['A'], symC = A.sym['C'], symG = A.sym['G'], symT = A.sym['T'];
    const uint32_t seg = (L + 63u) / 64u;
    const uint32_t s0 = (uint32_t)lane * seg, e0 = min(L, s0 + seg);
    uint32_t first = 0xFFFFFFFFu, ol_found = 0, pid = 0;
    if (s0 < L) {
        const uint32_t p0 = s0 >= A.max_pat_len ? s0 - A.max_pat_len : 0u;
        uint32_t state = 0, word = 0;
        for (uint32_t i = p0; i < e0; i++) {
            if ((i & 15u) == 0 || i == p0) word = g[i >> 4] >> ((i & 15u) * 2u);
            const uint32_t c = word & 3u;
            word >>= 2;
            if (A.go4) state = A.go4[state * 4 + c];
            else if (A.go4w) state = A.go4w[(size_t)state * 4 + c];
            else {
                const uint32_t sy = c == 0 ? symA : c == 1 ? symC : c == 2 ? symG : symT;
                state = A.go16 ? (uint32_t)A.go16[(size_t)state * A.n_sym1 + sy] : A.go32[(size_t)state * A.n_sym1 + sy];
            }
            if (i >= s0) {
                const uint32_t ol = A.out_len[state];
                if (ol) { first = i; ol_found = ol; pid = A.out_pid[state]; break; }
            }
        }
    }
    uint32_t best = first;
#pragma unroll
    for (int off = 32; off > 0; off >>= 1) best = min(best, (uint32_t)__shfl_xor((int)best, off));
    if (best == 0xFFFFFFFFu) { if (lane == 0) { info_by_slot[k] = 0; pid_by_slot[k] = 0; } return; }
    if (first == best) {
        info_by_slot[k] = ((best + 1) << 8) | ol_found;
        pid_by_slot[k] = pid;
    }
}

hipError_t launch_recruit_list(const DevReads &R, const DevAutomaton &A, const uint64_t *idx, const uint32_t *d_n,
                               uint64_t n_max, uint32_t *info_by_slot, uint32_t *pid_by_slot, hipStream_t st)
{
    if (n_max == 0) return hipSuccess;
    if (R.wave_walk && A.max_pat_len)
        CRASS_LAUNCH(k_recruit_list_wave, dim3((unsigned)((n_max + 3) / 4)), dim3(256), 0, st, R, A, idx, d_n, n_max, info_by_slot, pid_by_slot);
    else
        CRASS_LAUNCH(k_recruit_list, dim3((unsigned)((n_max + 255) / 256)), dim3(256), 0, st, R, A, idx, d_n, n_max, info_by_slot, pid_by_slot);
    return hipGetLastError();
}

__global__ __launch_bounds__(256) void k_recruit_exc(DevReads R, DevAutomaton A, const uint8_t *found_flag, uint32_t *exc_hit_info)
{
    uint64_t s = blockIdx.x * (uint64_t)blockDim.x + threadIdx.x;
    if (s >= R.n_exc) return;
    uint64_t r = R.exc_read[s];
    uint32_t info = 0;
    if (!found_flag[rd_header_id(R, r)]) {
        uint64_t o0 = R.exc_off[s];
        uint32_t L = (uint32_t)(R.exc_off[s + 1] - o0);
        uint32_t state = 0;
        for (uint32_t i = 0; i < L; i++) {
            uint32_t sy = A.sym[R.exc_bytes[o0 + i]];
            state = A.go16 ? (uint32_t)A.go16[(size_t)state * A.n_sym1 + sy] : A.go32[(size_t)state * A.n_sym1 + sy];
            uint32_t ol = A.out_len[state];
            if (ol) { info = ((i + 1) << 8) | ol; break; }
        }
    }
    exc_hit_info[s] = info;
}

hipError_t launch_recruit_exceptions(const DevReads &R, const DevAutomaton &A, const uint8_t *found_flag,
                                     uint32_t *exc_hit_info, hipStream_t st)
{
    if (R.n_exc == 0) return hipSuccess;
    CRASS_LAUNCH(k_recruit_exc, dim3((unsigned)((R.n_exc + 255) / 256)), dim3(256), 0, st, R, A, found_flag, exc_hit_info);
    return hipGetLastError();
}

template <bool EXC>
__global__ __launch_bounds__(256) void k_recruit_finish(DevReads R, const uint64_t *hit_idx, const uint32_t *d_n_hits,
                                                        uint64_t n_max, const uint32_t *hit_info, int info_by_slot,
                                                        const uint32_t *pid_by_slot, const uint32_t *pat_token,
                                                        RecruitOut *out, char *dr_chars, uint32_t dr_stride, const uint64_t *pat_mask)
{
    if constexpr (!EXC) CRASS_VGPR_FLOOR(24);
    uint64_t k = blockIdx.x * (uint64_t)blockDim.x + threadIdx.x;
    uint64_t n = EXC ? R.n_exc : (uint64_t)(*d_n_hits);
    if (n > n_max) n = n_max;
    if (k >= n) return;
    RecruitOut o; o.start = 0; o.end = 0; o.token = 0; o.dr_len = 0; o.low_lexi = 0; o.pad = 0;
    uint32_t info;
    uint32_t L;
    uint64_t r = 0, o0 = 0;
    const uint32_t *g = nullptr;
    if (EXC) {
        info = hit_info[k];
        o0 = R.exc_off[k];
        L = (uint32_t)(R.exc_off[k + 1] - o0);
    } else {
        r = hit_idx[k];
        info = info_by_slot ? hit_info[k] : hit_info[r];
        L = rd_len(R, r);
        g = R.packed + rd_word_off(R, r);
    }
    if (info == 0) { out[k] = o; return; }
    uint32_t textpos = info >> 8, len = info & 0xFFu;
    uint32_t DR_end = textpos - 1;
    if (DR_end >= L) DR_end = L - 1;
    uint32_t start = DR_end - (len - 1);
    const uint8_t *raw = nullptr;
    if (!EXC && pat_mask && pid_by_slot && pat_mask[pid_by_slot[k]] != 0ull && R.n_exc) {
        uint64_t lo = 0, hi = R.n_exc - 1;
        while (lo < hi) { const uint64_t mid = (lo + hi) >> 1; if (R.exc_read[mid] < r) lo = mid + 1; else hi = mid; }
        raw = R.exc_bytes + R.exc_off[lo];
    }
    if (!EXC && len <= 64 && !raw) {
        const uint32_t nw = (L + 15) >> 4, w0 = start >> 4, sh = (start & 15u) * 2u;
        uint32_t x[5];
#pragma unroll
        for (int q = 0; q < 5; q++) x[q] = (w0 + q < nw) ? g[w0 + q] : 0u;
        uint32_t y[4];
#pragma unroll
        for (int q = 0; q < 4; q++) y[q] = sh ? ((x[q] >> sh) | (x[q + 1] << (32 - sh))) : x[q];
        uint64_t v0 = (uint64_t)y[0] | ((uint64_t)y[1] << 32), v1 = (uint64_t)y[2] | ((uint64_t)y[3] << 32);
        const uint64_t m0 = len >= 32 ? ~0ull : ((1ull << (2 * len)) - 1ull);
        const uint64_t m1 = len >= 64 ? ~0ull : (len > 32 ? ((1ull << (2 * (len - 32))) - 1ull) : 0ull);
        v0 &= m0; v1 &= m1;
        auto rev2 = [](uint64_t t) -> uint64_t {
            t = __brevll(t);
            return ((t >> 1) & 0x5555555555555555ull) | ((t & 0x5555555555555555ull) << 1);
        };
        const uint64_t c0 = rev2(~v1), c1 = rev2(~v0);
        const uint32_t drop = 128u - 2u * len;
        uint64_t r0, r1;
        if (drop == 0) { r0 = c0; r1 = c1; }
        else if (drop < 64) { r0 = (c0 >> drop) | (c1 << (64 - drop)); r1 = c1 >> drop; }
        else { r0 = c1 >> (drop - 64); r1 = 0; }
        r0 &= m0; r1 &= m1;
        int less = 0;
        const uint64_t d0 = v0 ^ r0, d1 = v1 ^ r1;
        if (d0 | d1) {
            const uint64_t dv = d0 ? d0 : d1, av = d0 ? v0 : v1, bv = d0 ? r0 : r1;
            const int p = (__ffsll((unsigned long long)dv) - 1) & ~1;
            less = ((av >> p) & 3ull) < ((bv >> p) & 3ull);
        }
        const uint64_t s0 = less ? v0 : r0, s1 = less ? v1 : r1;
        if (dr_chars) {
            char *dr = dr_chars + k * (uint64_t)dr_stride;
            for (uint32_t i = 0; i < dr_stride; i++) {
                const uint32_t c = (uint32_t)(((i < 32 ? s0 : s1) >> (2 * (i & 31))) & 3ull);
                dr[i] = i < len ? "ACGT"[c] : (char)0;
            }
        }
        if (less) { o.start = start; o.end = DR_end; o.low_lexi = 1; }
        else { o.start = L - 1 - DR_end; o.end = L - 1 - start; o.low_lexi = 0; }
        o.dr_len = (uint16_t)len;
        if (pid_by_slot && pat_token) o.token = pat_token[pid_by_slot[k]];
        out[k] = o;
        return;
    }
    auto base_at = [&](uint32_t i) -> uint8_t {
        if (EXC) return R.exc_bytes[o0 + i];
        if (raw) return raw[i];
        uint32_t c = (g[i >> 4] >> ((i & 15u) * 2u)) & 3u;
        return (uint8_t)("ACGT"[c]);
    };
    int less = 0;
    for (uint32_t i = 0; i < len; i++) {
        uint8_t a = base_at(start + i);
        uint8_t b = c_comp.v[base_at(start + len - 1 - i) & 127];
        if (a != b) { less = a < b; break; }
    }
    char *dr = dr_chars ? dr_chars + k * (uint64_t)dr_stride : nullptr;
    if (less) {
        if (dr) for (uint32_t i = 0; i < len; i++) dr[i] = (char)base_at(start + i);
        o.start = start; o.end = DR_end; o.low_lexi = 1;
    } else {
        if (dr) for (uint32_t i = 0; i < len; i++) dr[i] = (char)c_comp.v[base_at(start + len - 1 - i) & 127];
        o.start = L - 1 - DR_end; o.end = L - 1 - start; o.low_lexi = 0;
    }
    if (dr) for (uint32_t i = len; i < dr_stride; i++) dr[i] = 0;
    o.dr_len = (uint16_t)len;
    if (pid_by_slot && pat_token) o.token = pat_token[pid_by_slot[k]];
    out[k] = o;
}

hipError_t launch_recruit_finish(const DevReads &R, const uint64_t *hit_idx, const uint32_t *d_n_hits, uint64_t n_hits_max,
                                 const uint32_t *hit_info, bool info_by_slot, bool exceptions,
                                 const uint32_t *pid_by_slot, const uint32_t *pat_token, RecruitOut *out,
                                 char *dr_chars, uint32_t dr_stride, hipStream_t st, const uint64_t *pat_mask)
{
    if (n_hits_max == 0) return hipSuccess;
    unsigned nb = (unsigned)((n_hits_max + 255) / 256);
    if (exceptions)
        CRASS_LAUNCH(k_recruit_finish<true>, dim3(nb), dim3(256), 0, st, R, hit_idx, d_n_hits, n_hits_max, hit_info, 1, pid_by_slot, pat_token, out, dr_chars, dr_stride, (const uint64_t *)nullptr);
    else
        CRASS_LAUNCH(k_recruit_finish<false>, dim3(nb), dim3(256), 0, st, R, hit_idx, d_n_hits, n_hits_max, hit_info, info_by_slot ? 1 : 0, pid_by_slot, pat_token, out, dr_chars, dr_stride, pat_mask);
    return hipGetLastError();
}

}
```

### crass_amd/csrc/sinks.hip

```cpp
#include "dev_common.h"
#include <algorithm>

namespace crass {

__global__ void k_build_exc_mask(const uint64_t *exc_read, uint64_t n_exc, uint32_t *exc_mask)
{
    uint64_t i = blockIdx.x * (uint64_t)blockDim.x + threadIdx.x;
    if (i < n_exc) {
        uint64_t r = exc_read[i];
        atomicOr(&exc_mask[r >> 5], 1u << (r & 31));
    }
}

__global__ void k_mark_found(const uint64_t *idx, uint64_t n, const uint64_t *header_id, uint8_t *found_flag)
{
    const uint64_t i = blockIdx.x * (uint64_t)blockDim.x + threadIdx.x;
    if (i < n) { const uint64_t r = idx[i]; found_flag[header_id ? header_id[r] : r] = 1; }
}
hipError_t launch_mark_found(const uint64_t *idx, uint64_t n, const uint64_t *header_id, uint8_t *found_flag, hipStream_t st)
{
    if (!n) return hipSuccess;
    CRASS_LAUNCH(k_mark_found, dim3((unsigned)((n + 255) / 256)), dim3(256), 0, st, idx, n, header_id, found_flag);
    return hipGetLastError();
}

__global__ __launch_bounds__(256) void k_copy_to_host(const uint4 *src, uint4 *dst, uint64_t n16, const uint8_t *src_tail, uint8_t *dst_tail, uint32_t n_tail)
{
    const uint64_t nth = (uint64_t)gridDim.x * blockDim.x;
    for (uint64_t i = blockIdx.x * (uint64_t)blockDim.x + threadIdx.x; i < n16; i += nth) dst[i] = src[i];
    if (blockIdx.x == 0 && threadIdx.x < n_tail) dst_tail[threadIdx.x] = src_tail[threadIdx.x];
}
hipError_t launch_copy_to_host(const void *d_src, void *h_dst, uint64_t bytes, hipStream_t st)
{
    if (!bytes) return hipSuccess;
    if ((reinterpret_cast<uintptr_t>(d_src) | reinterpret_cast<uintptr_t>(h_dst)) & 15u) return hipMemcpyAsync(h_dst, d_src, bytes, hipMemcpyDeviceToHost, st);
    const uint64_t n16 = bytes / 16;
    const unsigned blocks = (unsigned)std::min<uint64_t>(32, (n16 + 255) / 256 + 1);
    CRASS_LAUNCH(k_copy_to_host, dim3(blocks), dim3(256), 0, st, static_cast<const uint4 *>(d_src), static_cast<uint4 *>(h_dst), n16,
                 static_cast<const uint8_t *>(d_src) + n16 * 16, static_cast<uint8_t *>(h_dst) + n16 * 16, (uint32_t)(bytes & 15u));
    return hipGetLastError();
}

hipError_t launch_build_exc_mask(const uint64_t *exc_read, uint64_t n_exc, uint32_t *exc_mask, hipStream_t st)
{
    if (!n_exc) return hipSuccess;
    CRASS_LAUNCH(k_build_exc_mask, dim3((unsigned)((n_exc + 255) / 256)), dim3(256), 0, st, exc_read, n_exc, exc_mask);
    return hipGetLastError();
}

__global__ __launch_bounds__(256) void k_mask_count(const uint64_t *mask, uint64_t n_words, uint64_t n_bits,
                                                     uint32_t *word_prefix, uint32_t *block_sums)
{
    __shared__ uint32_t sh[256];
    uint64_t wi = blockIdx.x * 256ull + threadIdx.x;
    uint32_t c = 0;
    if (wi < n_words) {
        uint64_t m = mask[wi];
        uint64_t rem = n_bits - wi * 64;
        if (rem < 64) m &= (1ull << rem) - 1ull;
        c = (uint32_t)__popcll(m);
    }
    sh[threadIdx.x] = c;
    __syncthreads();
    for (int off = 1; off < 256; off <<= 1) {
        uint32_t v = (threadIdx.x >= (unsigned)off) ? sh[threadIdx.x - off] : 0;
        __syncthreads();
        sh[threadIdx.x] += v;
        __syncthreads();
    }
    if (wi < n_words) word_prefix[wi] = sh[threadIdx.x] - c;
    if (threadIdx.x == 255) block_sums[blockIdx.x] = sh[255];
}

__global__ __launch_bounds__(1024) void k_block_scan(uint32_t *block_sums, uint32_t n_blocks, uint32_t *d_count, uint32_t *zero_a, uint32_t n_a, uint32_t *zero_b, uint32_t n_b)
{
    if (threadIdx.x < n_a) zero_a[threadIdx.x] = 0u;
    if (threadIdx.x < n_b) zero_b[threadIdx.x] = 0u;

    __shared__ uint32_t sh[1024];
    __shared__ uint32_t carry;
    if (threadIdx.x == 0) carry = 0;
    __syncthreads();
    for (uint32_t base = 0; base < n_blocks; base += 1024) {
        uint32_t i = base + threadIdx.x;
        uint32_t c = (i < n_blocks) ? block_sums[i] : 0;
        sh[threadIdx.x] = c;
        __syncthreads();
        for (int off = 1; off < 1024; off <<= 1) {
            uint32_t v = (threadIdx.x >= (unsigned)off) ? sh[threadIdx.x - off] : 0;
            __syncthreads();
            sh[threadIdx.x] += v;
            __syncthreads();
        }
        uint32_t excl = sh[threadIdx.x] - c + carry;
        if (i < n_blocks) block_sums[i] = excl;
        __syncthreads();
        if (threadIdx.x == 1023) carry += sh[1023];
        __syncthreads();
    }
    if (threadIdx.x == 0) *d_count = carry;
}

__global__ __launch_bounds__(256) void k_mask_scatter(const uint64_t *mask, uint64_t n_words, uint64_t n_bits,
                                                       const uint32_t *word_prefix, const uint32_t *block_sums,
                                                       uint64_t *out_idx, uint64_t out_cap)
{
    uint64_t wi = blockIdx.x * 256ull + threadIdx.x;
    if (wi >= n_words) return;
    uint64_t m = mask[wi];
    uint64_t rem = n_bits - wi * 64;
    if (rem < 64) m &= (1ull << rem) - 1ull;
    uint64_t o = (uint64_t)block_sums[blockIdx.x] + word_prefix[wi];
    while (m) {
        int b = __ffsll((unsigned long long)m) - 1;
        m &= m - 1;
        if (o < out_cap) out_idx[o] = wi * 64 + b;
        o++;
    }
}

static __device__ __forceinline__ unsigned long long lb_pack(uint32_t epoch, uint32_t flag, uint32_t value)
{
    return ((unsigned long long)epoch << 34) | ((unsigned long long)flag << 32) | value;
}
static __device__ uint32_t lb_exclusive_prefix(const Lookback &lb, uint32_t tile, uint32_t total)
{
    __shared__ uint32_t excl_sh;
    if (threadIdx.x < 64) {
        const int lane = (int)threadIdx.x;
        if (lane == 0)
            __hip_atomic_store(&lb.status[tile], lb_pack(lb.epoch, tile == 0 ? 2u : 1u, total), __ATOMIC_RELAXED, __HIP_MEMORY_SCOPE_AGENT);
        uint32_t excl = 0;
        int t = (int)tile - 1;
        while (t >= 0) {
            const int idx = t - lane;
            uint32_t flag = 2u, val = 0u;
            if (idx >= 0) {
                flag = 0u;
                for (uint32_t spins = 0; spins < (1u << 24); spins++) {
                    const unsigned long long w = __hip_atomic_load(&lb.status[idx], __ATOMIC_RELAXED, __HIP_MEMORY_SCOPE_AGENT);
                    if ((uint32_t)(w >> 34) == lb.epoch && ((w >> 32) & 3ull) != 0ull) { flag = (uint32_t)(w >> 32) & 3u; val = (uint32_t)w; break; }
                    __builtin_amdgcn_s_sleep(1);
                }
                if (flag == 0u) { *lb.fail = 1u; flag = 2u; }
            }
            const unsigned long long pm = __ballot(flag == 2u);
            const int stop = pm ? __ffsll(pm) - 1 : 64;
            uint32_t v = lane <= stop ? val : 0u;
#pragma unroll
            for (int off = 32; off > 0; off >>= 1) v += (uint32_t)__shfl_xor((int)v, off);
            excl += v;
            if (pm) break;
            t -= 64;
        }
        if (lane == 0) {
            if (tile != 0) __hip_atomic_store(&lb.status[tile], lb_pack(lb.epoch, 2u, excl + total), __ATOMIC_RELAXED, __HIP_MEMORY_SCOPE_AGENT);
            excl_sh = excl;
        }
    }
    __syncthreads();
    return excl_sh;
}
static __device__ uint32_t lb_tile_id(const Lookback &lb, uint32_t n_act)
{
    __shared__ uint32_t tile_sh;
    if (threadIdx.x == 0) {
        const uint32_t t = atomicAdd(lb.ticket, 1u);
        if (t + 1u >= n_act) __hip_atomic_store(lb.ticket, 0u, __ATOMIC_RELAXED, __HIP_MEMORY_SCOPE_AGENT);
        tile_sh = t;
    }
    __syncthreads();
    return tile_sh;
}
template <int T>
static __device__ uint32_t block_scan_t(uint32_t v, uint32_t *total)
{
    __shared__ uint32_t wsum[T / 64];
    const int lane = threadIdx.x & 63, wv = threadIdx.x >> 6;
    uint32_t incl = v;
#pragma unroll
    for (int off = 1; off < 64; off <<= 1) {
        const uint32_t y = (uint32_t)__shfl_up((int)incl, off);
        if (lane >= off) incl += y;
    }
    if (lane == 63) wsum[wv] = incl;
    __syncthreads();
    uint32_t base = 0, all = 0;
#pragma unroll
    for (int k = 0; k < T / 64; k++) { const uint32_t s = wsum[k]; if (k < wv) base += s; all += s; }
    *total = all;
    return base + incl - v;
}

template <int T, int W>
__global__ __launch_bounds__(T) void k_mask_compact_lb(const uint64_t *mask, uint64_t n_words, uint64_t n_bits, uint32_t *word_prefix,
                                                        uint32_t *block_sums, uint64_t *out_idx, uint64_t out_cap, uint32_t *d_count,
                                                        uint32_t *zero_a, uint32_t n_a, uint32_t *zero_b, uint32_t n_b, Lookback lb,
                                                        uint32_t n_tiles)
{
    const uint32_t tile = lb_tile_id(lb, n_tiles);
    if (tile == 0) {
        if (threadIdx.x < n_a) zero_a[threadIdx.x] = 0u;
        if (threadIdx.x < n_b) zero_b[threadIdx.x] = 0u;
    }
    const uint64_t w0 = ((uint64_t)tile * T + threadIdx.x) * W;
    uint64_t m[W];
    uint32_t cnt = 0;
#pragma unroll
    for (int q = 0; q < W; q++) {
        const uint64_t wi = w0 + q;
        m[q] = 0;
        if (wi < n_words) {
            m[q] = mask[wi];
            const uint64_t rem = n_bits - wi * 64;
            if (rem < 64) m[q] &= (1ull << rem) - 1ull;
        }
        cnt += (uint32_t)__popcll(m[q]);
    }
    uint32_t total;
    const uint32_t in_tile = block_scan_t<T>(cnt, &total);
    const uint32_t excl = lb_exclusive_prefix(lb, tile, total);
    if (tile == n_tiles - 1 && threadIdx.x == 0) *d_count = excl + total;
    uint64_t o = (uint64_t)excl + in_tile;
#pragma unroll
    for (int q = 0; q < W; q++) {
        const uint64_t wi = w0 + q;
        if (wi >= n_words) break;
        if (word_prefix) {
            word_prefix[wi] = (uint32_t)o;
            if ((wi & 255u) == 0) block_sums[wi >> 8] = 0u;
        }
        uint64_t mm = m[q];
        while (mm) {
            const int b = __ffsll((unsigned long long)mm) - 1;
            mm &= mm - 1;
            if (o < out_cap) out_idx[o] = wi * 64 + b;
            o++;
        }
    }
}

static constexpr uint32_t kLbElemsPerTile = 4096;
static __device__ uint32_t lb_rank4(const Lookback &lb, uint32_t tile, uint32_t cnt, uint32_t *upto)
{
    uint32_t all;
    const uint32_t in_tile = block_scan_t<1024>(cnt, &all);
    const uint32_t excl = lb_exclusive_prefix(lb, tile, all);
    *upto = excl + all;
    return excl + in_tile;
}

hipError_t launch_compact(const uint64_t *mask, uint64_t n_words, uint64_t n_bits, uint32_t *word_prefix,
                          uint32_t *block_sums, uint64_t *out_idx, uint64_t out_cap, uint32_t *d_count, hipStream_t st,
                          uint32_t *zero_a, uint32_t n_a, uint32_t *zero_b, uint32_t n_b, const Lookback *lb)
{
    if (lb && n_words) {
        const uint32_t tw = lookback_tile_words(n_words);
        const uint32_t n_tiles = (uint32_t)((n_words + tw - 1) / tw);
        if (tw == 256)
            CRASS_LAUNCH((k_mask_compact_lb<256, 1>), dim3(n_tiles), dim3(256), 0, st, mask, n_words, n_bits, word_prefix, block_sums, out_idx, out_cap,
                               d_count, zero_a, n_a, zero_b, n_b, *lb, n_tiles);
        else
            CRASS_LAUNCH((k_mask_compact_lb<1024, 4>), dim3(n_tiles), dim3(1024), 0, st, mask, n_words, n_bits, word_prefix, block_sums, out_idx, out_cap,
                               d_count, zero_a, n_a, zero_b, n_b, *lb, n_tiles);
        return hipGetLastError();
    }
    if (n_words == 0) {
        if (n_a) (void)hipMemsetAsync(zero_a, 0, 4 * (size_t)n_a, st);
        if (n_b) (void)hipMemsetAsync(zero_b, 0, 4 * (size_t)n_b, st);
        return hipMemsetAsync(d_count, 0, 4, st);
    }
    unsigned nb = (unsigned)((n_words + 255) / 256);
    CRASS_LAUNCH(k_mask_count, dim3(nb), dim3(256), 0, st, mask, n_words, n_bits, word_prefix, block_sums);
    CRASS_LAUNCH(k_block_scan, dim3(1), dim3(1024), 0, st, block_sums, nb, d_count, zero_a, n_a, zero_b, n_b);
    CRASS_LAUNCH(k_mask_scatter, dim3(nb), dim3(256), 0, st, mask, n_words, n_bits, word_prefix, block_sums, out_idx, out_cap);
    return hipGetLastError();
}

__global__ __launch_bounds__(256) void k_found_mask(const SurvOut *out, const uint32_t *d_n, uint64_t n, uint64_t *mask, uint32_t *d_err,
                                                     unsigned long long *dd_keys, uint32_t *dd_first, uint32_t dd_size)
{
    const uint64_t s = blockIdx.x * (uint64_t)blockDim.x + threadIdx.x;
    for (uint64_t i = s; i < dd_size; i += (uint64_t)gridDim.x * blockDim.x) { dd_keys[i] = 0ull; dd_first[i] = 0xFFFFFFFFu; }
    bool f = false;
    if (s < n && s < (uint64_t)*d_n) {
        const SurvOut o = out[s];
        f = o.found != 0;
        if (o.err) atomicMax(d_err, (uint32_t)o.err);
    }
    const uint64_t m = __ballot(f);
    if ((threadIdx.x & 63) == 0 && s < n) mask[s >> 6] = m;
}

static __device__ uint64_t dr_hash64(const char *p, uint32_t n)
{
    uint64_t h = 0x9E3779B97F4A7C15ull ^ ((uint64_t)n * 0xD6E8FEB86659FD93ull);
    while (n >= 8) {
        uint64_t v = 0;
        for (int i = 0; i < 8; i++) v |= (uint64_t)(uint8_t)p[i] << (8 * i);
        h = (h ^ v) * 0xFF51AFD7ED558CCDull; h ^= h >> 32; p += 8; n -= 8;
    }
    if (n) {
        uint64_t v = 0;
        for (uint32_t i = 0; i < n; i++) v |= (uint64_t)(uint8_t)p[i] << (8 * i);
        h = (h ^ v) * 0xC4CEB9FE1A85EC53ull; h ^= h >> 29;
    }
    return h ^ (h >> 31);
}

#define GF_BLOCK 1024
#define GF_SLOTS 2048
__global__ __launch_bounds__(GF_BLOCK) void k_gather_found(const uint64_t *fidx, const uint32_t *d_nf, uint64_t n_max,
                                                            const SurvOut *out, const uint64_t *surv_idx, uint64_t read_base,
                                                            const char *dr_chars, uint32_t dr_stride, const uint32_t *ss_pool,
                                                            uint32_t ss_cap, uint32_t ss_elem, uint8_t *blob, uint16_t *g_dr_len, char *g_dr,
                                                            unsigned long long *dd_keys, uint32_t *dd_first, uint32_t dd_mask,
                                                            uint64_t *dd_hash, uint32_t *dd_slot, uint32_t *d_mismatch)
{
    __shared__ unsigned long long lkey[GF_SLOTS];
    __shared__ uint32_t lmin[GF_SLOTS], lslot[GF_SLOTS];
    const uint64_t k = blockIdx.x * (uint64_t)GF_BLOCK + threadIdx.x;
    uint64_t n = *d_nf;
    if (n > n_max) n = n_max;
    if (blockIdx.x * (uint64_t)GF_BLOCK >= n) return;
    if (dd_keys) {
        for (uint32_t i = threadIdx.x; i < GF_SLOTS; i += GF_BLOCK) { lkey[i] = 0ull; lmin[i] = 0xFFFFFFFFu; }
        __syncthreads();
    }
    uint32_t ls = 0;
    if (k < n) {
        const P1Blob b = p1_blob_layout(n, ss_cap, ss_elem);
        const uint64_t s = fidx[k];
// ... 324 lines not shown
            }
            if (!same) atomicOr(d_mismatch, 1u);
        }
    }
    uint32_t all;
    const uint32_t in_tile = block_scan_t<1024>(is_rep ? 1u : 0u, &all);
    const uint32_t excl = lb_exclusive_prefix(lb, tile, all);
    if (tile == n_tiles - 1 && threadIdx.x == 0) *d_nd = excl + all;
    if (is_rep) { const uint32_t q = excl + in_tile; dx_idx[q] = k; slot_of[k] = q; }
}

__global__ __launch_bounds__(256) void k_dx_assign_gather(const uint32_t *rep, const uint32_t *d_n, uint32_t n_max, const uint32_t *rank_of,
                                                           uint32_t *dmap, const uint64_t *dx_idx, const uint32_t *d_nd, const char *dr,
                                                           const uint16_t *dr_len, const uint64_t *hash, uint32_t stride, char *out_chars,
                                                           uint16_t *out_len, uint64_t *out_hash, char *dev_chars, uint16_t *dev_len,
                                                           const uint32_t *cnt_src, uint32_t *cnt_dst, uint32_t n_cnt)
{
    const uint32_t j = blockIdx.x * blockDim.x + threadIdx.x;
    if (j < n_cnt) cnt_dst[j] = cnt_src[j];
    if (j < min(*d_n, n_max)) dmap[j] = rank_of[rep[j]];
    uint32_t nd = *d_nd;
    if (nd > n_max) nd = n_max;
    if (j >= nd) return;
    const uint64_t k = dx_idx[j];
    const uint4 *src = reinterpret_cast<const uint4 *>(dr + k * stride);
    uint4 *dst = reinterpret_cast<uint4 *>(out_chars + (uint64_t)j * stride);
    uint4 *dst2 = reinterpret_cast<uint4 *>(dev_chars + (uint64_t)j * stride);
    for (uint32_t i = 0; i < stride / 16; i++) { const uint4 v = src[i]; if (out_chars) dst[i] = v; if (dev_chars) dst2[i] = v; }
    const uint16_t l = dr_len[k];
    if (out_len) out_len[j] = l;
    if (dev_len) dev_len[j] = l;
    if (out_hash) out_hash[j] = hash[k];
}

hipError_t launch_dx_tokens(const char *dr, const uint16_t *dr_len, const uint64_t *hash, uint32_t stride, const uint32_t *d_n, uint32_t n, uint32_t *rep,
                            uint32_t *slot_of, const uint32_t *first,
                            uint64_t *mask, uint32_t *word_prefix, uint32_t *block_sums, uint64_t *dx_idx, uint32_t *d_nd,
                            uint32_t *d_mismatch, uint32_t *dmap, char *out_chars, uint16_t *out_len, uint64_t *out_hash,
                            char *dev_chars, uint16_t *dev_len, hipStream_t st, const uint32_t *cnt_src, uint32_t *cnt_dst, uint32_t n_cnt,
                            const Lookback *lb)
{
    if (n == 0) return hipSuccess;
    const unsigned nb = (n + 255) / 256;
    if (lb) {
        const uint32_t n_tiles = (n + 1023u) / 1024u;
        CRASS_LAUNCH(k_dx_flag_compact, dim3(n_tiles), dim3(1024), 0, st, dr, dr_len, stride, d_n, n, slot_of, first, rep, dx_idx, d_nd, d_mismatch,
                           *lb);
        CRASS_LAUNCH(k_dx_assign_gather, dim3(nb), dim3(256), 0, st, rep, d_n, n, (const uint32_t *)slot_of, dmap, dx_idx, d_nd, dr, dr_len,
                           hash, stride, out_chars, out_len, out_hash, dev_chars, dev_len, cnt_src, cnt_dst, cnt_dst ? n_cnt : 0u);
        return hipGetLastError();
    }
    CRASS_LAUNCH(k_dx_flag, dim3(nb), dim3(256), 0, st, dr, dr_len, stride, d_n, n, slot_of, first, rep, mask, d_mismatch);
    hipError_t e = launch_compact(mask, (n + 63) / 64, n, word_prefix, block_sums, dx_idx, n, d_nd, st);
    if (e != hipSuccess) return e;
    CRASS_LAUNCH(k_dx_assign, dim3(nb), dim3(256), 0, st, rep, d_n, n, mask, word_prefix, block_sums, dmap);
    CRASS_LAUNCH(k_dx_gather, dim3(nb), dim3(256), 0, st, dx_idx, d_nd, n, dr, dr_len, hash, stride, out_chars, out_len, out_hash, dev_chars, dev_len,
                       cnt_src, cnt_dst, cnt_dst ? n_cnt : 0u);
    return hipGetLastError();
}

__global__ __launch_bounds__(256) void k_recruit_valid_mask(const RecruitOut *rec, const uint32_t *d_n, uint64_t n_max, uint64_t *mask)
{
    const uint64_t k = blockIdx.x * (uint64_t)blockDim.x + threadIdx.x;
    uint64_t n = *d_n;
    if (n > n_max) n = n_max;
    const bool v = k < n && rec[k].dr_len != 0;
    const uint64_t m = __ballot(v);
    if ((threadIdx.x & 63) == 0 && k < n_max) mask[k >> 6] = m;
}
__global__ __launch_bounds__(256) void k_pack_p2_blob(const RecruitOut *rec, const uint64_t *hit_idx, uint64_t read_base, const uint64_t *vidx,
                                                       const uint32_t *d_nv, uint64_t cap, uint8_t *blob, const uint32_t *d_n_hits, uint32_t *h_n_hits,
                                                       uint32_t narrow)
{
    const uint64_t q = blockIdx.x * (uint64_t)blockDim.x + threadIdx.x;
    uint64_t nv = *d_nv;
    if (nv > cap) nv = cap;
    if (q == 0) {
        reinterpret_cast<uint64_t *>(blob)[0] = nv; reinterpret_cast<uint64_t *>(blob)[1] = cap;
        if (h_n_hits) *h_n_hits = *d_n_hits;
    }
    if (q >= nv) return;
    const P2Blob b = p2_blob_layout(cap, narrow);
    const uint64_t k = vidx[q];
    const RecruitOut o = rec[k];
    if (narrow == 2) {
        reinterpret_cast<uint32_t *>(blob + b.token)[q] = o.token | ((uint32_t)(o.low_lexi != 0) << 31);
        reinterpret_cast<uint32_t *>(blob + b.read)[q] = (uint32_t)hit_idx[k];
        (blob + b.start)[q] = (uint8_t)o.start;
        return;
    }
    reinterpret_cast<uint32_t *>(blob + b.token)[q] = o.token;
    if (narrow) {
        reinterpret_cast<uint32_t *>(blob + b.read)[q] = (uint32_t)hit_idx[k];
        (blob + b.start)[q] = (uint8_t)o.start;
        (blob + b.end)[q] = (uint8_t)o.end;
    } else {
        reinterpret_cast<uint64_t *>(blob + b.read)[q] = read_base + hit_idx[k];
        reinterpret_cast<uint16_t *>(blob + b.start)[q] = (uint16_t)o.start;
        reinterpret_cast<uint16_t *>(blob + b.end)[q] = (uint16_t)o.end;
    }
    (blob + b.dr_len)[q] = (uint8_t)o.dr_len;
    (blob + b.low)[q] = o.low_lexi;
}
__global__ __launch_bounds__(1024) void k_valid_compact(const RecruitOut *rec, const uint32_t *d_n_hits, uint64_t cap, uint64_t *vidx, uint32_t *d_nv,
                                                         Lookback lb)
{
    uint64_t n = *d_n_hits;
    if (n > cap) n = cap;
    const uint32_t n_tiles = n ? (uint32_t)((n + kLbElemsPerTile - 1) / kLbElemsPerTile) : 1u;
    if (blockIdx.x >= n_tiles) return;
    const uint32_t tile = lb_tile_id(lb, n_tiles);
    const uint64_t k0 = (uint64_t)tile * kLbElemsPerTile + 4u * threadIdx.x;
    uint32_t fm = 0;
#pragma unroll
    for (int e = 0; e < 4; e++) if (k0 + e < n && rec[k0 + e].dr_len != 0) fm |= 1u << e;
    uint32_t upto;
    uint64_t q = lb_rank4(lb, tile, (uint32_t)__popc(fm), &upto);
    if (tile == n_tiles - 1 && threadIdx.x == 0) *d_nv = upto;
#pragma unroll
    for (int e = 0; e < 4; e++) if (fm & (1u << e)) vidx[q++] = k0 + e;
}

hipError_t launch_pack_p2_blob(const RecruitOut *rec, const uint64_t *hit_idx, uint64_t read_base,
                               const uint32_t *d_n_hits, uint64_t n_hits_max, uint64_t *mask, uint32_t *word_prefix, uint32_t *block_sums,
                               uint64_t *vidx, uint32_t *d_nv, uint8_t *blob, hipStream_t st, uint32_t *h_n_hits, const Lookback *lb, uint32_t narrow)
{
    if (n_hits_max == 0) return hipSuccess;
    const unsigned nb = (unsigned)((n_hits_max + 255) / 256);
    if (lb) {
        const unsigned nt = (unsigned)((n_hits_max + kLbElemsPerTile - 1) / kLbElemsPerTile);
        CRASS_LAUNCH(k_valid_compact, dim3(nt), dim3(1024), 0, st, rec, d_n_hits, n_hits_max, vidx, d_nv, *lb);
        CRASS_LAUNCH(k_pack_p2_blob, dim3(nb), dim3(256), 0, st, rec, hit_idx, read_base, vidx, d_nv, n_hits_max, blob, d_n_hits, h_n_hits, narrow);
        return hipGetLastError();
    }
    CRASS_LAUNCH(k_recruit_valid_mask, dim3(nb), dim3(256), 0, st, rec, d_n_hits, n_hits_max, mask);
    hipError_t e = launch_compact(mask, (n_hits_max + 63) / 64, n_hits_max, word_prefix, block_sums, vidx, n_hits_max, d_nv, st);
    if (e != hipSuccess) return e;
    CRASS_LAUNCH(k_pack_p2_blob, dim3(nb), dim3(256), 0, st, rec, hit_idx, read_base, vidx, d_nv, n_hits_max, blob, d_n_hits, h_n_hits, narrow);
    return hipGetLastError();
}

}
```

Before: 29.83 billion reads/s.

## Fuse pass-2 recruit finish with blob packing and chunk tail across streams

Adds a fused kernel that compacts verified hits with a decoupled lookback scan, runs recruit_finish per surviving slot, and writes straight into the pass-2 host blob. This removes the intermediate RecruitOut buffer and the separate pack and compaction launches. Optionally the verify and pack stages are split into chunks, with packing on a side stream carrying counts between chunks, so packing can overlap later verify work. The cost is more complex cross-stream synchronisation and lookback state per chunk.

```diff
diff --git a/crass_amd/build.py b/crass_amd/build.py
--- a/crass_amd/build.py
+++ b/crass_amd/build.py
@@ -7,7 +7,7 @@
 CSRC = os.path.join(HERE, "csrc")
 LIB = os.path.join(HERE, "libcrass_hip.so")
 SOURCES = ["kernels.hip", "pass2.hip", "sinks.hip", "dmerge.hip", "consensus.hip", "pack.hip", "fastx_scan.hip", "fastx_names.hip", "inflate.hip", "gunzip.hip", "engine.cpp", "engine_pass1.cpp", "engine_merge.cpp", "engine_pass2.cpp", "engine_ingest.cpp", "merge.cpp", "ingest.cpp", "fastx_scan.cpp", "bgzf.cpp", "gunzip.cpp", "consensus.cpp", "group.cpp", "graph.cpp", "sdma.cpp", "pgzip.cpp"]
-HEADERS = ["engine_internal.h", "engine_ctx.h", "dev_common.h", "comp_table.h", "devmem.h", "pack_text.h", "lane_find.h", "pack_launch.h", "fastx_scan.h", "fastx_launch.h", "fastx_shards.h", "fastx_names_launch.h", "inflate_core.h", "inflate_launch.h", "gunzip_core.h", "gunzip_launch.h", "consensus_internal.h", "merge.h", os.path.join("..", "..", "include", "crass_hip.h")]
+HEADERS = ["engine_internal.h", "engine_ctx.h", "dev_common.h", "lookback.h", "comp_table.h", "devmem.h", "pack_text.h", "lane_find.h", "pack_launch.h", "fastx_scan.h", "fastx_launch.h", "fastx_shards.h", "fastx_names_launch.h", "inflate_core.h", "inflate_launch.h", "gunzip_core.h", "gunzip_launch.h", "consensus_internal.h", "merge.h", os.path.join("..", "..", "include", "crass_hip.h")]
 
 
 def _hipcc():
diff --git a/crass_amd/csrc/dev_common.h b/crass_amd/csrc/dev_common.h
--- a/crass_amd/csrc/dev_common.h
+++ b/crass_amd/csrc/dev_common.h
@@ -37,6 +37,29 @@
     return R.header_id ? R.header_id[r] : r;
 }
 
+static __device__ __forceinline__ void p2_blob_store(uint8_t *blob, const P2Blob &b, uint64_t q, const RecruitOut &o, uint64_t read_local,
+                                                     uint64_t read_base)
+{
+    if (b.narrow == 2) {
+        reinterpret_cast<uint32_t *>(blob + b.token)[q] = o.token | ((uint32_t)(o.low_lexi != 0) << 31);
+        reinterpret_cast<uint32_t *>(blob + b.read)[q] = (uint32_t)read_local;
+        (blob + b.start)[q] = (uint8_t)o.start;
+        return;
+    }
+    reinterpret_cast<uint32_t *>(blob + b.token)[q] = o.token;
+    if (b.narrow) {
+        reinterpret_cast<uint32_t *>(blob + b.read)[q] = (uint32_t)read_local;
+        (blob + b.start)[q] = (uint8_t)o.start;
+        (blob + b.end)[q] = (uint8_t)o.end;
+    } else {
+        reinterpret_cast<uint64_t *>(blob + b.read)[q] = read_base + read_local;
+        reinterpret_cast<uint16_t *>(blob + b.start)[q] = (uint16_t)o.start;
+        reinterpret_cast<uint16_t *>(blob + b.end)[q] = (uint16_t)o.end;
+    }
+    (blob + b.dr_len)[q] = (uint8_t)o.dr_len;
+    (blob + b.low)[q] = o.low_lexi;
+}
+
 typedef unsigned short u16x2 __attribute__((ext_vector_type(2)));
 static __device__ __forceinline__ uint32_t pk_min_u16(uint32_t a, uint32_t b)
 {
diff --git a/crass_amd/csrc/dmerge.hip b/crass_amd/csrc/dmerge.hip
--- a/crass_amd/csrc/dmerge.hip
+++ b/crass_amd/csrc/dmerge.hip
@@ -941,7 +941,7 @@
 
 template <bool SHORT, int U>
 __global__ __launch_bounds__(256) void k_dm_verify(DevReads R, DevMerge M, const uint64_t *idx, const uint32_t *d_n, uint64_t n_max,
-                                                    uint32_t *info_by_slot, uint32_t *pid_by_slot)
+                                                    uint32_t *info_by_slot, uint32_t *pid_by_slot, uint64_t k_lo)
 {
     __shared__ uint32_t rw_all[4][DV_G][DV_MAXW + 2];
     const int lane = threadIdx.x & 63, wv = threadIdx.x >> 6;
@@ -949,6 +949,8 @@
     const uint64_t n_waves = ((uint64_t)gridDim.x * blockDim.x) >> 6;
     uint64_t n = *d_n;
     if (n > n_max) n = n_max;
+    n = n > k_lo ? n - k_lo : 0;
+    idx += k_lo; info_by_slot += k_lo; pid_by_slot += k_lo;
     const uint32_t kmask = (1u << M.kset_log) - 1u;
     if (SHORT) {
         const int gi = lane / DV_GL, pl = lane % DV_GL;
@@ -1122,17 +1124,18 @@
 }
 
 hipError_t launch_dm_verify(const DevReads &R, const DevMerge &M, const uint64_t *idx, const uint32_t *d_n, uint64_t n_max,
-                            uint32_t *info_by_slot, uint32_t *pid_by_slot, hipStream_t st)
-{
-    if (n_max == 0) return hipSuccess;
+                            uint32_t *info_by_slot, uint32_t *pid_by_slot, hipStream_t st, uint64_t k_lo)
+{
+    if (n_max <= k_lo) return hipSuccess;
+    const uint64_t n_rng = n_max - k_lo;
     static const bool dv_one = getenv("CRASS_DV_ONE") != nullptr;
     const bool shortr = M.akey_shift == 3 && M.akey_bases == 16 && R.uniform_len >= 16 && ((R.uniform_len - 16) >> 3) < DV_GL && ((R.uniform_len + 15) >> 4) <= DV_MAXW && !dv_one;
-    uint64_t nb = shortr ? (n_max + 4 * DV_G - 1) / (4 * DV_G) : (n_max + 3) / 4;
+    uint64_t nb = shortr ? (n_rng + 4 * DV_G - 1) / (4 * DV_G) : (n_rng + 3) / 4;
     if (nb > 8192) nb = 8192;
     static const bool dv_pair = getenv("CRASS_DV_SINGLE") == nullptr;
-    if (shortr && dv_pair) CRASS_LAUNCH((k_dm_verify<true, 2>), dim3((unsigned)nb), dim3(256), 0, st, R, M, idx, d_n, n_max, info_by_slot, pid_by_slot);
-    else if (shortr) CRASS_LAUNCH((k_dm_verify<true, 1>), dim3((unsigned)nb), dim3(256), 0, st, R, M, idx, d_n, n_max, info_by_slot, pid_by_slot);
-    else CRASS_LAUNCH((k_dm_verify<false, 1>), dim3((unsigned)nb), dim3(256), 0, st, R, M, idx, d_n, n_max, info_by_slot, pid_by_slot);
+    if (shortr && dv_pair) CRASS_LAUNCH((k_dm_verify<true, 2>), dim3((unsigned)nb), dim3(256), 0, st, R, M, idx, d_n, n_max, info_by_slot, pid_by_slot, k_lo);
+    else if (shortr) CRASS_LAUNCH((k_dm_verify<true, 1>), dim3((unsigned)nb), dim3(256), 0, st, R, M, idx, d_n, n_max, info_by_slot, pid_by_slot, k_lo);
+    else CRASS_LAUNCH((k_dm_verify<false, 1>), dim3((unsigned)nb), dim3(256), 0, st, R, M, idx, d_n, n_max, info_by_slot, pid_by_slot, k_lo);
     return hipGetLastError();
 }
 
diff --git a/crass_amd/csrc/engine.cpp b/crass_amd/csrc/engine.cpp
--- a/crass_amd/csrc/engine.cpp
+++ b/crass_amd/csrc/engine.cpp
@@ -224,6 +224,9 @@
     for (auto &d : c->dma_sink) { sdma_destroy(d); d = nullptr; }
     for (auto &d : c->dma_dx) { sdma_destroy(d); d = nullptr; }
     if (c->ev_premerge) (void)hipEventDestroy(c->ev_premerge);
+    for (auto &e : c->ev_tail) if (e) (void)hipEventDestroy(e);
+    if (c->ev_tail_done) (void)hipEventDestroy(c->ev_tail_done);
+    c->tail_carry.release();
     if (c->copy_stream) (void)hipStreamDestroy(c->copy_stream);
     c->r_packed.release(); c->r_word_off.release(); c->r_lengths.release(); c->r_header_id.release();
     c->r_exc_mask.release(); c->r_exc_read.release(); c->r_exc_off.release(); c->r_exc_bytes.release();
diff --git a/crass_amd/csrc/engine_ctx.h b/crass_amd/csrc/engine_ctx.h
--- a/crass_amd/csrc/engine_ctx.h
+++ b/crass_amd/csrc/engine_ctx.h
@@ -237,6 +237,8 @@
     bool inflate_hbm_window = true;
     uint32_t hid_hash_bits = 64;
     bool lane_find_serial = false;
+    bool p2_tail_serial = false;
+    uint32_t p2_tail_chunks = 0;
     uint32_t probe_blocks = 0;
     void read()
     {
@@ -263,6 +265,8 @@
         hid_hash_bits = 64; if (const char *e = getenv("CRASS_HID_TEST_HASH_BITS")) hid_hash_bits = (uint32_t)std::min(64, std::max(0, atoi(e)));
         lane_find_serial = false; if (const char *e = getenv("CRASS_LANE_FIND_SERIAL")) lane_find_serial = atoi(e) != 0;
         probe_blocks = 0; if (const char *e = getenv("CRASS_PROBE_BLOCKS")) probe_blocks = (uint32_t)std::max(0, atoi(e));
+        p2_tail_serial = false; if (const char *e = getenv("CRASS_P2_TAIL_SERIAL")) p2_tail_serial = atoi(e) != 0;
+        p2_tail_chunks = 0; if (const char *e = getenv("CRASS_P2_TAIL_CHUNKS")) p2_tail_chunks = (uint32_t)std::min(16, std::max(0, atoi(e)));
         pool_cap_bytes = 0; if (const char *e = getenv("CRASS_POOL_CAP_MB")) pool_cap_bytes = (uint64_t)std::max(1ll, atoll(e)) << 20;
     }
 };
@@ -351,6 +355,11 @@
     uint64_t hit_cap_hint = 0;
     bool recruit_exact = false;
     hipStream_t copy_stream = nullptr;
+    static constexpr uint32_t kTailMaxChunks = 16;
+    hipEvent_t ev_tail[kTailMaxChunks] = {}, ev_tail_done = nullptr;
+    DevBuf<uint32_t> tail_carry;
+    bool tail_fused() const { return !env.p2_tail_serial && lb_on; }
+    bool tail_on_side = false;
     static constexpr int kHintParts = 4;
     hipStream_t hint_stream = nullptr;
     hipEvent_t ev_hint[kHintParts] = {nullptr, nullptr, nullptr, nullptr}, ev_hint_go = nullptr;
diff --git a/crass_amd/csrc/engine_internal.h b/crass_amd/csrc/engine_internal.h
--- a/crass_amd/csrc/engine_internal.h
+++ b/crass_amd/csrc/engine_internal.h
@@ -227,7 +227,8 @@
                                hipEvent_t ev_apply = nullptr);
 hipError_t launch_anchor_filter_dev(const DevReads &R, const DevMerge &M, const uint8_t *found_flag, uint64_t *hitmask, hipStream_t st, uint32_t max_blocks = 0);
 hipError_t launch_dm_verify(const DevReads &R, const DevMerge &M, const uint64_t *idx, const uint32_t *d_n, uint64_t n_max,
-                            uint32_t *info_by_slot, uint32_t *pid_by_slot, hipStream_t st);
+                            uint32_t *info_by_slot, uint32_t *pid_by_slot, hipStream_t st,
+                            uint64_t k_lo = 0);
 hipError_t warm_dmerge_module();
 
 struct SurvLds {
@@ -320,6 +321,10 @@
                                  const uint32_t *pid_by_slot, const uint32_t *pat_token,
                                  RecruitOut *out, char *dr_chars, uint32_t dr_stride, hipStream_t st,
                                  const uint64_t *pat_mask = nullptr);
+hipError_t launch_finish_pack_p2(const DevReads &R, const uint64_t *hit_idx, const uint32_t *d_n_hits, uint64_t k_lo, uint64_t k_hi, uint64_t cap,
+                                 const uint32_t *info_by_slot, const uint32_t *pid_by_slot, const uint32_t *pat_token, const uint64_t *pat_mask,
+                                 uint64_t read_base, uint8_t *blob, uint32_t narrow, const uint32_t *carry_in, uint32_t *carry_out, bool last,
+                                 uint32_t *h_n_hits, const Lookback &lb, hipStream_t st);
 hipError_t launch_levenshtein_batch(const uint8_t *chars, const uint64_t *a_off, const uint32_t *a_len,
                                     const uint64_t *b_off, const uint32_t *b_len, uint64_t n_pairs,
                                     int32_t *dist, float *sim, uint32_t max_len, hipStream_t st);
diff --git a/crass_amd/csrc/engine_pass1.cpp b/crass_amd/csrc/engine_pass1.cpp
--- a/crass_amd/csrc/engine_pass1.cpp
+++ b/crass_amd/csrc/engine_pass1.cpp
@@ -537,7 +537,7 @@
 {
     const uint64_t s_alloc = h_alloc + n_exc;
     { const int ms = ensure_mask_scratch(c, h_alloc); if (ms) return ms; }
-    HIPCHK(c, c->d_rec.ensure(s_alloc + 1));
+    if (!dev_sink || !c->tail_fused()) HIPCHK(c, c->d_rec.ensure(s_alloc + 1));
     HIPCHK(c, c->d_dr.ensure((s_alloc + 1) * c->dr_stride));
     if (!dev_sink) {
         HIPCHK(c, c->h_rec.ensure(s_alloc + 1));
diff --git a/crass_amd/csrc/engine_pass2.cpp b/crass_amd/csrc/engine_pass2.cpp
--- a/crass_amd/csrc/engine_pass2.cpp
+++ b/crass_amd/csrc/engine_pass2.cpp
@@ -54,14 +54,66 @@
     return CRASS_OK;
 }
 
-static int recruit_device_sink(crass_hip_ctx *c, bool spec, uint64_t n_hits, const uint64_t *extra_found, uint64_t n_extra)
+static uint32_t p2_narrow(const crass_hip_ctx *c)
 {
     static const bool blob12 = getenv("CRASS_P2_BLOB12") != nullptr;
-    const uint32_t narrow = (c->max_len <= 255 && c->R.n_reads < (1ull << 32)) ? ((blob12 || c->host_view_light) ? 1u : 2u) : 0u;
+    return (c->max_len <= 255 && c->R.n_reads < (1ull << 32)) ? ((blob12 || c->host_view_light) ? 1u : 2u) : 0u;
+}
+
+static constexpr uint64_t kTailChunkAlign = 1024;
+static int queue_fused_tail(crass_hip_ctx *c, bool spec, uint64_t n_hits, bool &queued)
+{
+    queued = false;
+    const uint32_t want = c->env.p2_tail_chunks ? c->env.p2_tail_chunks : 1u;
+    const uint64_t expect = spec ? (2 * n_hits + 2) / 3 : n_hits;
+    const uint64_t step = std::max<uint64_t>(((expect + want - 1) / want + kTailChunkAlign - 1) & ~(kTailChunkAlign - 1), kTailChunkAlign);
+    uint64_t edge[crass_hip_ctx::kTailMaxChunks + 1];
+    uint32_t n_ch = 0;
+    for (uint64_t k = 0; k < n_hits && n_ch < want; k += step) edge[n_ch++] = k;
+    edge[n_ch] = n_hits;
+    Lookback lb[crass_hip_ctx::kTailMaxChunks];
+    c->prealloc_lookback((n_hits + 4095) / 4096);
+    for (uint32_t i = 0; i < n_ch; i++) if (!c->next_lookback_elems(edge[i + 1] - edge[i], &lb[i])) return CRASS_OK;
+    HIPCHK(c, c->tail_carry.ensure(crass_hip_ctx::kTailMaxChunks + 1));
+    const bool side = n_ch > 1;
+    hipStream_t fs = side ? c->copy_stream : c->stream;
+    const uint32_t narrow = p2_narrow(c);
+    for (uint32_t i = 0; i < n_ch; i++) {
+        HIPCHK(c, launch_dm_verify(c->R, c->dm.M, c->d_idx.p, c->d_count.p, edge[i + 1], c->d_slot_info.p, c->d_slot_pid.p, c->stream, edge[i]));
+        if (side) {
+            if (!c->ev_tail[i]) HIPCHK(c, hipEventCreateWithFlags(&c->ev_tail[i], hipEventDisableTiming));
+            HIPCHK(c, hipEventRecord(c->ev_tail[i], c->stream));
+            HIPCHK(c, hipStreamWaitEvent(fs, c->ev_tail[i], 0));
+            lb[i].ticket = c->lb_ticket.p + 1;
+        }
+        HIPCHK(c, launch_finish_pack_p2(c->R, c->d_idx.p, c->d_count.p, edge[i], edge[i + 1], n_hits, c->d_slot_info.p, c->d_slot_pid.p, c->dm.M.pat_token,
+                                        c->dm.M.pat_mask, c->read_base, c->h_qblob.p, narrow, i ? c->tail_carry.p + i : nullptr, c->tail_carry.p + i + 1,
+                                        i + 1 == n_ch, spec ? c->h_count.p : nullptr, lb[i], fs));
+    }
+    c->tail_on_side = side;
+    if (side && c->timed(7, 2)) {
+        if (!c->ev_tail_done) HIPCHK(c, hipEventCreateWithFlags(&c->ev_tail_done, hipEventDisableTiming));
+        HIPCHK(c, hipEventRecord(c->ev_tail_done, fs));
+        HIPCHK(c, hipStreamWaitEvent(c->stream, c->ev_tail_done, 0));
+    }
+    queued = true;
+    return CRASS_OK;
+}
+static hipError_t sync_tail(crass_hip_ctx *c)
+{
+    const hipError_t e = hipStreamSynchronize(c->stream);
+    if (e != hipSuccess || !c->tail_on_side) return e;
+    return hipStreamSynchronize(c->copy_stream);
+}
+
+static int recruit_device_sink(crass_hip_ctx *c, bool spec, uint64_t n_hits, bool fused, const uint64_t *extra_found, uint64_t n_extra)
+{
+    const uint32_t narrow = p2_narrow(c);
     c->q_lay = p2_blob_layout(n_hits, narrow);
     c->q_wide_ready = false;
     Lookback lbq;
-    if (n_hits) {
+    if (fused) ;
+    else if (n_hits) {
         HIPCHK(c, launch_pack_p2_blob(c->d_rec.p, c->d_idx.p, c->read_base, c->d_count.p, n_hits, c->d_mask.p,
                                       c->d_word_prefix.p, c->d_block_sums.p, c->d_fidx.p, c->d_count.p + 6, c->h_qblob.p, c->stream,
                                       spec ? c->h_count.p : nullptr, c->next_lookback_elems(n_hits, &lbq), narrow));
@@ -73,11 +125,11 @@
         fprintf(stderr, "[crass_dm] recruit: tail queued %.1f us after the pass-1 sync, then blocked %.1f us on the host view\n",
                 1e3 * (th0 - c->t_p1_sync), 1e3 * (now_ms() - th0));
     if (hs == CRASS_ERR_STATE) {
-        HIPCHK(c, hipStreamSynchronize(c->stream));
+        HIPCHK(c, sync_tail(c));
         return recruit_after_host_merge(c, extra_found, n_extra);
     }
     if (hs) return hs;
-    HIPCHK(c, hipStreamSynchronize(c->stream));
+    HIPCHK(c, sync_tail(c));
     if (c->env.merge_profile)
         fprintf(stderr, "[crass_dm] recruit: final synchronisation returned %.1f us after the pass-1 sync\n", 1e3 * (now_ms() - c->t_p1_sync));
     if (spec) {
@@ -186,6 +238,14 @@
     const uint64_t n_hits = spec ? c->hit_cap_hint : c->h_count.p[0];
     const uint64_t h_alloc = spec ? n_hits : std::max<uint64_t>(n_hits, hit_bound(n_hits));
     { const int as = ensure_recruit_buffers(c, h_alloc, n_exc, dmp, anchors); if (as) return as; }
+    bool fused = false;
+    c->tail_on_side = false;
+    if (dmp && n_hits && c->tail_fused()) { const int ts = queue_fused_tail(c, spec, n_hits, fused); if (ts) return ts; }
+    if (fused) {
+        HIPCHK(c, c->stamp(7, 2));
+        return recruit_device_sink(c, spec, n_hits, true, extra_found, n_extra);
+    }
+    HIPCHK(c, c->d_rec.ensure(n_hits + n_exc + 1));
     if (anchors) {
         if (dmp) HIPCHK(c, launch_dm_verify(c->R, c->dm.M, c->d_idx.p, c->d_count.p, n_hits, c->d_slot_info.p, c->d_slot_pid.p, c->stream));
         else HIPCHK(c, launch_recruit_list(c->R, c->A, c->d_idx.p, c->d_count.p, n_hits, c->d_slot_info.p, c->d_slot_pid.p, c->stream));
@@ -198,7 +258,7 @@
         HIPCHK(c, launch_recruit_finish(c->R, nullptr, nullptr, n_exc, c->d_exc_hit.p, true, true, nullptr, nullptr, c->d_rec.p + n_hits,
                                         c->d_dr.p + n_hits * c->dr_stride, c->dr_stride, c->stream));
     HIPCHK(c, c->stamp(7, 2));
-    if (dmp) return recruit_device_sink(c, spec, n_hits, extra_found, n_extra);
+    if (dmp) return recruit_device_sink(c, spec, n_hits, false, extra_found, n_extra);
     return recruit_host_sink(c, n_hits, n_exc, anchors, lds);
 }
 
diff --git a/crass_amd/csrc/lookback.h b/crass_amd/csrc/lookback.h
--- /dev/null
+++ b/crass_amd/csrc/lookback.h
@@ -0,0 +1,84 @@
+#pragma once
+
+static __device__ __forceinline__ unsigned long long lb_pack(uint32_t epoch, uint32_t flag, uint32_t value)
+{
+    return ((unsigned long long)epoch << 34) | ((unsigned long long)flag << 32) | value;
+}
+static __device__ uint32_t lb_exclusive_prefix(const Lookback &lb, uint32_t tile, uint32_t total)
+{
+    __shared__ uint32_t excl_sh;
+    if (threadIdx.x < 64) {
+        const int lane = (int)threadIdx.x;
+        if (lane == 0)
+            __hip_atomic_store(&lb.status[tile], lb_pack(lb.epoch, tile == 0 ? 2u : 1u, total), __ATOMIC_RELAXED, __HIP_MEMORY_SCOPE_AGENT);
+        uint32_t excl = 0;
+        int t = (int)tile - 1;
+        while (t >= 0) {
+            const int idx = t - lane;
+            uint32_t flag = 2u, val = 0u;
+            if (idx >= 0) {
+                flag = 0u;
+                for (uint32_t spins = 0; spins < (1u << 24); spins++) {
+                    const unsigned long long w = __hip_atomic_load(&lb.status[idx], __ATOMIC_RELAXED, __HIP_MEMORY_SCOPE_AGENT);
+                    if ((uint32_t)(w >> 34) == lb.epoch && ((w >> 32) & 3ull) != 0ull) { flag = (uint32_t)(w >> 32) & 3u; val = (uint32_t)w; break; }
+                    __builtin_amdgcn_s_sleep(1);
+                }
+                if (flag == 0u) { *lb.fail = 1u; flag = 2u; }
+            }
+            const unsigned long long pm = __ballot(flag == 2u);
+            const int stop = pm ? __ffsll(pm) - 1 : 64;
+            uint32_t v = lane <= stop ? val : 0u;
+#pragma unroll
+            for (int off = 32; off > 0; off >>= 1) v += (uint32_t)__shfl_xor((int)v, off);
+            excl += v;
+            if (pm) break;
+            t -= 64;
+        }
+        if (lane == 0) {
+            if (tile != 0) __hip_atomic_store(&lb.status[tile], lb_pack(lb.epoch, 2u, excl + total), __ATOMIC_RELAXED, __HIP_MEMORY_SCOPE_AGENT);
+            excl_sh = excl;
+        }
+    }
+    __syncthreads();
+    return excl_sh;
+}
+static __device__ uint32_t lb_tile_id(const Lookback &lb, uint32_t n_act)
+{
+    __shared__ uint32_t tile_sh;
+    if (threadIdx.x == 0) {
+        const uint32_t t = atomicAdd(lb.ticket, 1u);
+        if (t + 1u >= n_act) __hip_atomic_store(lb.ticket, 0u, __ATOMIC_RELAXED, __HIP_MEMORY_SCOPE_AGENT);
+        tile_sh = t;
+    }
+    __syncthreads();
+    return tile_sh;
+}
+template <int T>
+static __device__ uint32_t block_scan_t(uint32_t v, uint32_t *total)
+{
+    __shared__ uint32_t wsum[T / 64];
+    const int lane = threadIdx.x & 63, wv = threadIdx.x >> 6;
+    uint32_t incl = v;
+#pragma unroll
+    for (int off = 1; off < 64; off <<= 1) {
+        const uint32_t y = (uint32_t)__shfl_up((int)incl, off);
+        if (lane >= off) incl += y;
+    }
+    if (lane == 63) wsum[wv] = incl;
+    __syncthreads();
+    uint32_t base = 0, all = 0;
+#pragma unroll
+    for (int k = 0; k < T / 64; k++) { const uint32_t s = wsum[k]; if (k < wv) base += s; all += s; }
+    *total = all;
+    return base + incl - v;
+}
+
+static constexpr uint32_t kLbElemsPerTile = 4096;
+static __device__ uint32_t lb_rank4(const Lookback &lb, uint32_t tile, uint32_t cnt, uint32_t *upto)
+{
+    uint32_t all;
+    const uint32_t in_tile = block_scan_t<1024>(cnt, &all);
+    const uint32_t excl = lb_exclusive_prefix(lb, tile, all);
+    *upto = excl + all;
+    return excl + in_tile;
+}
diff --git a/crass_amd/csrc/pass2.hip b/crass_amd/csrc/pass2.hip
--- a/crass_amd/csrc/pass2.hip
+++ b/crass_amd/csrc/pass2.hip
@@ -4,6 +4,8 @@
 #include <utility>
 
 namespace crass {
+
+#include "lookback.h"
 
 static __constant__ CompTable c_comp = make_comp_table();
 
@@ -530,32 +532,22 @@
 }
 
 template <bool EXC>
-__global__ __launch_bounds__(256) void k_recruit_finish(DevReads R, const uint64_t *hit_idx, const uint32_t *d_n_hits,
-                                                        uint64_t n_max, const uint32_t *hit_info, int info_by_slot,
-                                                        const uint32_t *pid_by_slot, const uint32_t *pat_token,
-                                                        RecruitOut *out, char *dr_chars, uint32_t dr_stride, const uint64_t *pat_mask)
-{
-    if constexpr (!EXC) CRASS_VGPR_FLOOR(24);
-    uint64_t k = blockIdx.x * (uint64_t)blockDim.x + threadIdx.x;
-    uint64_t n = EXC ? R.n_exc : (uint64_t)(*d_n_hits);
-    if (n > n_max) n = n_max;
-    if (k >= n) return;
+static __device__ __forceinline__ RecruitOut recruit_finish_slot(const DevReads &R, uint64_t k, uint64_t r, uint32_t info,
+                                                                 const uint32_t *pid_by_slot, const uint32_t *pat_token,
+                                                                 char *dr_chars, uint32_t dr_stride, const uint64_t *pat_mask)
+{
     RecruitOut o; o.start = 0; o.end = 0; o.token = 0; o.dr_len = 0; o.low_lexi = 0; o.pad = 0;
-    uint32_t info;
+    if (info == 0) return o;
     uint32_t L;
-    uint64_t r = 0, o0 = 0;
+    uint64_t o0 = 0;
     const uint32_t *g = nullptr;
     if (EXC) {
-        info = hit_info[k];
         o0 = R.exc_off[k];
         L = (uint32_t)(R.exc_off[k + 1] - o0);
     } else {
-        r = hit_idx[k];
-        info = info_by_slot ? hit_info[k] : hit_info[r];
         L = rd_len(R, r);
         g = R.packed + rd_word_off(R, r);
     }
-    if (info == 0) { out[k] = o; return; }
     uint32_t textpos = info >> 8, len = info & 0xFFu;
     uint32_t DR_end = textpos - 1;
     if (DR_end >= L) DR_end = L - 1;
@@ -608,8 +600,7 @@
         else { o.start = L - 1 - DR_end; o.end = L - 1 - start; o.low_lexi = 0; }
         o.dr_len = (uint16_t)len;
         if (pid_by_slot && pat_token) o.token = pat_token[pid_by_slot[k]];
-        out[k] = o;
-        return;
+        return o;
     }
     auto base_at = [&](uint32_t i) -> uint8_t {
         if (EXC) return R.exc_bytes[o0 + i];
@@ -634,7 +625,78 @@
     if (dr) for (uint32_t i = len; i < dr_stride; i++) dr[i] = 0;
     o.dr_len = (uint16_t)len;
     if (pid_by_slot && pat_token) o.token = pat_token[pid_by_slot[k]];
-    out[k] = o;
+    return o;
+}
+
+template <bool EXC>
+__global__ __launch_bounds__(256) void k_recruit_finish(DevReads R, const uint64_t *hit_idx, const uint32_t *d_n_hits,
+                                                        uint64_t n_max, const uint32_t *hit_info, int info_by_slot,
+                                                        const uint32_t *pid_by_slot, const uint32_t *pat_token,
+                                                        RecruitOut *out, char *dr_chars, uint32_t dr_stride, const uint64_t *pat_mask)
+{
+    if constexpr (!EXC) CRASS_VGPR_FLOOR(24);
+    uint64_t k = blockIdx.x * (uint64_t)blockDim.x + threadIdx.x;
+    uint64_t n = EXC ? R.n_exc : (uint64_t)(*d_n_hits);
+    if (n > n_max) n = n_max;
+    if (k >= n) return;
+    const uint64_t r = EXC ? 0 : hit_idx[k];
+    const uint32_t info = (EXC || info_by_slot) ? hit_info[k] : hit_info[r];
+    out[k] = recruit_finish_slot<EXC>(R, k, r, info, pid_by_slot, pat_token, dr_chars, dr_stride, pat_mask);
+}
+
+__global__ __launch_bounds__(1024) void k_finish_pack_p2(DevReads R, const uint64_t *hit_idx, const uint32_t *d_n_hits, uint64_t k_lo, uint64_t k_hi,
+                                                          uint64_t cap, const uint32_t *info_by_slot, const uint32_t *pid_by_slot,
+                                                          const uint32_t *pat_token, const uint64_t *pat_mask, uint64_t read_base,
+                                                          uint8_t *blob, uint32_t narrow, const uint32_t *carry_in, uint32_t *carry_out,
+                                                          int last, uint32_t *h_n_hits, Lookback lb)
+{
+    constexpr int T = 1024, E = 4;
+    constexpr uint32_t kTile = kLbElemsPerTile;
+    __shared__ uint16_t slot_of_rank[kTile];
+    uint64_t n_end = *d_n_hits;
+    if (n_end > k_hi) n_end = k_hi;
+    const uint64_t n = n_end > k_lo ? n_end - k_lo : 0;
+    const uint32_t n_tiles = n ? (uint32_t)((n + kTile - 1) / kTile) : 1u;
+    if (blockIdx.x >= n_tiles) return;
+    const uint32_t tile = lb_tile_id(lb, n_tiles);
+    const uint64_t t0 = k_lo + (uint64_t)tile * kTile;
+    const uint32_t e0 = (uint32_t)E * threadIdx.x;
+    uint32_t fm = 0;
+#pragma unroll
+    for (int e = 0; e < E; e++) if (t0 + e0 + e < n_end && info_by_slot[t0 + e0 + e] != 0u) fm |= 1u << e;
+    uint32_t all;
+    uint32_t in_tile = block_scan_t<T>((uint32_t)__popc(fm), &all);
+    const uint32_t excl = lb_exclusive_prefix(lb, tile, all);
+    const uint32_t before = (carry_in ? *carry_in : 0u) + excl;
+#pragma unroll
+    for (int e = 0; e < E; e++) if (fm & (1u << e)) slot_of_rank[in_tile++] = (uint16_t)(e0 + e);
+    __syncthreads();
+    if (tile == n_tiles - 1 && threadIdx.x == 0) {
+        *carry_out = before + all;
+        if (last) {
+            reinterpret_cast<uint64_t *>(blob)[0] = before + all; reinterpret_cast<uint64_t *>(blob)[1] = cap;
+            if (h_n_hits) *h_n_hits = *d_n_hits;
+        }
+    }
+    const P2Blob b = p2_blob_layout(cap, narrow);
+    for (uint32_t j = threadIdx.x; j < all; j += (uint32_t)T) {
+        const uint64_t k = t0 + slot_of_rank[j];
+        const uint64_t r = hit_idx[k];
+        const RecruitOut o = recruit_finish_slot<false>(R, k, r, info_by_slot[k], pid_by_slot, pat_token, nullptr, 0, pat_mask);
+        p2_blob_store(blob, b, (uint64_t)before + j, o, r, read_base);
+    }
+}
+
+hipError_t launch_finish_pack_p2(const DevReads &R, const uint64_t *hit_idx, const uint32_t *d_n_hits, uint64_t k_lo, uint64_t k_hi, uint64_t cap,
+                                 const uint32_t *info_by_slot, const uint32_t *pid_by_slot, const uint32_t *pat_token, const uint64_t *pat_mask,
+                                 uint64_t read_base, uint8_t *blob, uint32_t narrow, const uint32_t *carry_in, uint32_t *carry_out, bool last,
+                                 uint32_t *h_n_hits, const Lookback &lb, hipStream_t st)
+{
+    if (k_hi <= k_lo) return hipErrorInvalidValue;
+    const unsigned nt = (unsigned)((k_hi - k_lo + kLbElemsPerTile - 1) / kLbElemsPerTile);
+    CRASS_LAUNCH(k_finish_pack_p2, dim3(nt), dim3(1024), 0, st, R, hit_idx, d_n_hits, k_lo, k_hi, cap, info_by_slot, pid_by_slot, pat_token, pat_mask,
+                 read_base, blob, narrow, carry_in, carry_out, last ? 1 : 0, h_n_hits, lb);
+    return hipGetLastError();
 }
 
 hipError_t launch_recruit_finish(const DevReads &R, const uint64_t *hit_idx, const uint32_t *d_n_hits, uint64_t n_hits_max,
diff --git a/crass_amd/csrc/sinks.hip b/crass_amd/csrc/sinks.hip
--- a/crass_amd/csrc/sinks.hip
+++ b/crass_amd/csrc/sinks.hip
@@ -2,6 +2,8 @@
 #include <algorithm>
 
 namespace crass {
+
+#include "lookback.h"
 
 __global__ void k_build_exc_mask(const uint64_t *exc_read, uint64_t n_exc, uint32_t *exc_mask)
 {
@@ -119,79 +121,6 @@
     }
 }
 
-static __device__ __forceinline__ unsigned long long lb_pack(uint32_t epoch, uint32_t flag, uint32_t value)
-{
-    return ((unsigned long long)epoch << 34) | ((unsigned long long)flag << 32) | value;
-}
-static __device__ uint32_t lb_exclusive_prefix(const Lookback &lb, uint32_t tile, uint32_t total)
-{
-    __shared__ uint32_t excl_sh;
-    if (threadIdx.x < 64) {
-        const int lane = (int)threadIdx.x;
-        if (lane == 0)
-            __hip_atomic_store(&lb.status[tile], lb_pack(lb.epoch, tile == 0 ? 2u : 1u, total), __ATOMIC_RELAXED, __HIP_MEMORY_SCOPE_AGENT);
-        uint32_t excl = 0;
-        int t = (int)tile - 1;
-        while (t >= 0) {
-            const int idx = t - lane;
-            uint32_t flag = 2u, val = 0u;
-            if (idx >= 0) {
-                flag = 0u;
-                for (uint32_t spins = 0; spins < (1u << 24); spins++) {
-                    const unsigned long long w = __hip_atomic_load(&lb.status[idx], __ATOMIC_RELAXED, __HIP_MEMORY_SCOPE_AGENT);
-                    if ((uint32_t)(w >> 34) == lb.epoch && ((w >> 32) & 3ull) != 0ull) { flag = (uint32_t)(w >> 32) & 3u; val = (uint32_t)w; break; }
-                    __builtin_amdgcn_s_sleep(1);
-                }
-                if (flag == 0u) { *lb.fail = 1u; flag = 2u; }
-            }
-            const unsigned long long pm = __ballot(flag == 2u);
-            const int stop = pm ? __ffsll(pm) - 1 : 64;
-            uint32_t v = lane <= stop ? val : 0u;
-#pragma unroll
-            for (int off = 32; off > 0; off >>= 1) v += (uint32_t)__shfl_xor((int)v, off);
-            excl += v;
-            if (pm) break;
-            t -= 64;
-        }
-        if (lane == 0) {
-            if (tile != 0) __hip_atomic_store(&lb.status[tile], lb_pack(lb.epoch, 2u, excl + total), __ATOMIC_RELAXED, __HIP_MEMORY_SCOPE_AGENT);
-            excl_sh = excl;
-        }
-    }
-    __syncthreads();
-    return excl_sh;
-}
-static __device__ uint32_t lb_tile_id(const Lookback &lb, uint32_t n_act)
-{
-    __shared__ uint32_t tile_sh;
-    if (threadIdx.x == 0) {
-        const uint32_t t = atomicAdd(lb.ticket, 1u);
-        if (t + 1u >= n_act) __hip_atomic_store(lb.ticket, 0u, __ATOMIC_RELAXED, __HIP_MEMORY_SCOPE_AGENT);
-        tile_sh = t;
-    }
-    __syncthreads();
-    return tile_sh;
-}
-template <int T>
-static __device__ uint32_t block_scan_t(uint32_t v, uint32_t *total)
-{
-    __shared__ uint32_t wsum[T / 64];
-    const int lane = threadIdx.x & 63, wv = threadIdx.x >> 6;
-    uint32_t incl = v;
-#pragma unroll
-    for (int off = 1; off < 64; off <<= 1) {
-        const uint32_t y = (uint32_t)__shfl_up((int)incl, off);
-        if (lane >= off) incl += y;
-    }
-    if (lane == 63) wsum[wv] = incl;
-    __syncthreads();
-    uint32_t base = 0, all = 0;
-#pragma unroll
-    for (int k = 0; k < T / 64; k++) { const uint32_t s = wsum[k]; if (k < wv) base += s; all += s; }
-    *total = all;
-    return base + incl - v;
-}
-
 template <int T, int W>
 __global__ __launch_bounds__(T) void k_mask_compact_lb(const uint64_t *mask, uint64_t n_words, uint64_t n_bits, uint32_t *word_prefix,
                                                         uint32_t *block_sums, uint64_t *out_idx, uint64_t out_cap, uint32_t *d_count,
@@ -238,16 +167,6 @@
             o++;
         }
     }
-}
-
-static constexpr uint32_t kLbElemsPerTile = 4096;
-static __device__ uint32_t lb_rank4(const Lookback &lb, uint32_t tile, uint32_t cnt, uint32_t *upto)
-{
-    uint32_t all;
-    const uint32_t in_tile = block_scan_t<1024>(cnt, &all);
-    const uint32_t excl = lb_exclusive_prefix(lb, tile, all);
-    *upto = excl + all;
-    return excl + in_tile;
 }
 
 hipError_t launch_compact(const uint64_t *mask, uint64_t n_words, uint64_t n_bits, uint32_t *word_prefix,
@@ -738,25 +657,7 @@
     if (q >= nv) return;
     const P2Blob b = p2_blob_layout(cap, narrow);
     const uint64_t k = vidx[q];
-    const RecruitOut o = rec[k];
-    if (narrow == 2) {
-        reinterpret_cast<uint32_t *>(blob + b.token)[q] = o.token | ((uint32_t)(o.low_lexi != 0) << 31);
-        reinterpret_cast<uint32_t *>(blob + b.read)[q] = (uint32_t)hit_idx[k];
-        (blob + b.start)[q] = (uint8_t)o.start;
-        return;
-    }
-    reinterpret_cast<uint32_t *>(blob + b.token)[q] = o.token;
-    if (narrow) {
-        reinterpret_cast<uint32_t *>(blob + b.read)[q] = (uint32_t)hit_idx[k];
-        (blob + b.start)[q] = (uint8_t)o.start;
-        (blob + b.end)[q] = (uint8_t)o.end;
-    } else {
-        reinterpret_cast<uint64_t *>(blob + b.read)[q] = read_base + hit_idx[k];
-        reinterpret_cast<uint16_t *>(blob + b.start)[q] = (uint16_t)o.start;
-        reinterpret_cast<uint16_t *>(blob + b.end)[q] = (uint16_t)o.end;
-    }
-    (blob + b.dr_len)[q] = (uint8_t)o.dr_len;
-    (blob + b.low)[q] = o.low_lexi;
+    p2_blob_store(blob, b, q, rec[k], hit_idx[k], read_base);
 }
 __global__ __launch_bounds__(1024) void k_valid_compact(const RecruitOut *rec, const uint32_t *d_n_hits, uint64_t cap, uint64_t *vidx, uint32_t *d_nv,
                                                          Lookback lb)
```

Measured after the change: 29.77 billion reads/s. About the same (-0.2%).
